# Lqm26/BMCNet-ESR

Measured on AMD Instinct MI355X. Metric: LR-voxel-frames/sec x4 SR train step, NFS-shaped 180x240 (BASELINE configs[1] / [2]), f32, higher is better.
Workload: dtype f32; 1 GPU; BMCNet(scale=4, n_c=128, n_b=5) x4 SR train step, NFS-shaped 180x240 (BASELINE configs[1] / [2]) -> 720x960, bs=4/GPU, arithmetic fp32 (native fp32 MFMA; 3x3 convolutions through Winograd F(4x4,3x3) / F(2x2,3x3) transforms in fp32), SEQL=9 SEQN=2 (8 windows BPTT), event scatter + fwd + MSE + bwd + Adam(amsgrad); global_batch=4, parallelism=dp1, rccl_ranks=1, rccl_initialised_before_headline_run=False

## Files before the change

### bmcnet-esr_amd/bmc_hip/bie.py

```python
from __future__ import annotations

import ctypes as C
import os
import weakref

import torch

from . import lib, ops
from .ops import ConvSpec, _dense_spec, _need_gpu, _null_src, _src, _stream, conv_launch, dgrad_launch, pgemm_raw, round_up

_SPEC2 = {}

FUSE_CHAIN = os.environ.get("BMC_FUSE_CHAIN", "1") != "0"
_CHAIN_CACHE = {}



VFREE = os.environ.get("BMC_BIE_VFREE", "1") != "0"
VFREE_MIN_PIXELS = int(os.environ.get("BMC_BIE_VFREE_MIN_PIXELS", 1 << 16))


def vfree_supported(npx):
    return VFREE and ops.MATH in (0, 3) and npx >= VFREE_MIN_PIXELS


def _gram_on_x(c_src, x_src, B, H, W, Cn, dev):
    slabs, nsplit, G, bsl = pgemm_raw(c_src, [x_src], B, H, W, 1, 1, Cn, Cn, dev, flops=2.0 * B * H * W * Cn * Cn, want_bias=True)
    G0 = torch.empty((B, Cn, Cn), device=dev, dtype=torch.float32)
    sc = torch.empty((B, Cn), device=dev, dtype=torch.float32)
    lib.call(lib._red_w, "bmc_pgemm_reduce_weight", slabs.data_ptr(), nsplit, G, 1, Cn, Cn, None, Cn, G0.data_ptr(), 0,
             bsl.data_ptr(), sc.data_ptr(), _stream())
    return G0, sc


def _times_wt(m, vec, wg, bg, bpg, alpha, out):
    B, Cn, _ = m.shape
    ops.small_mm([((m, Cn * Cn, 0, Cn, 1), (wg, 0, Cn * Cn, 1, Cn), None)], B, bpg, Cn, Cn, Cn, c=(out, Cn * Cn, 0, Cn, 1),
                 alpha=alpha, uv=((vec, Cn, 0), (bg, 0, Cn)))
    return out


def _times_w(m, wg, bg, bpg, out, out_strides, vec=None):
    B, Cn, _ = m.shape
    ops.small_mm([((m, Cn * Cn, 0, Cn, 1), (wg, 0, Cn * Cn, Cn, 1), (bg, 0, Cn, 1) if vec is not None else None)], B, bpg, Cn, Cn, Cn,
                 c=(out, out_strides[0], 0, out_strides[1], out_strides[2]), vec_out=(vec, Cn, 0) if vec is not None else None)


def _value_param_grads(p, dM, tg, da, G0, sc, w_params, b_params, npx):
    groups = len(w_params)
    B, Cn, _ = p.shape
    n, cc, dev = B // groups, Cn * Cn, p.device
    mp = round_up(Cn, 32)
    slab, bslab = groups * mp * mp, groups * 4 * mp
    slabs = torch.empty(n * slab, device=dev, dtype=torch.float32)
    bsl = torch.zeros(n * bslab, device=dev, dtype=torch.float32)
    params = list(w_params) + list(b_params)
    with ops.wgrad_side(npx, params, (p, dM, tg, da, G0, sc)):
        ops._on_side(slabs, bsl)
        ops.small_mm([((p, cc, 0, 1, Cn), (dM, cc, 0, Cn, 1), (tg, Cn, 0, 1)), ((da, cc, 0, 1, Cn), (G0, cc, 0, Cn, 1), (sc, Cn, 0, 1))],
                     B, n, Cn, Cn, Cn, c=(slabs, slab, mp * mp - n * slab, mp, 1), vec_out=(bsl, bslab, 4 * mp - n * bslab))
        one = groups == 1
        return ops.reduce_wgrad(slabs, n, groups, 1, Cn, _dense_spec(Cn), dev, bsl, w_params[0] if one else tuple(w_params),
                                b_params[0] if one else tuple(b_params), (Cn, Cn) if one else (groups, Cn, Cn))


def chain_supported(Cn):
    return FUSE_CHAIN and ops.MATH in (0, 3) and Cn in (32, 64, 128)


def _chain_streams(wf, wc, Cn):
    key = (id(wf), id(wc))
    hit = _CHAIN_CACHE.get(key)
    if hit is not None and hit[0]() is wf and hit[1]() is wc and hit[2] == (wf._version, wc._version):
        return hit[3], hit[4]
    dev = wf.device
    s1, s2 = _dense_spec(Cn), _spec2(Cn)
    st = _stream()

    def pack(w, spec, cin):
        out = torch.empty(spec.kpad * Cn, device=dev, dtype=torch.float32)
        lib.call(lib._pack_w, "bmc_pack_weight", w.data_ptr(), spec.kmap(dev).data_ptr(), 1, Cn, cin, 1, spec.kpad, Cn,
                 out.data_ptr(), st)
        return out

    def pack_t(w, spec, cin, src_index):
        out = torch.empty(Cn * Cn, device=dev, dtype=torch.float32)
        lib.call(lib._pack_wt, "bmc_pack_weight_t", w.data_ptr(), spec.kmap(dev).data_ptr(), 1, Cn, cin, 1,
                 src_index * Cn, Cn, Cn, Cn, out.data_ptr(), st)
        return out

    wfd, wcd = wf.detach().contiguous(), wc.detach().contiguous()
    fwd = torch.cat([pack(wfd, s2, 2 * Cn), pack(wcd, s1, Cn)])
    tc, t0, t1 = pack_t(wcd, s1, Cn, 0), pack_t(wfd, s2, 2 * Cn, 0), pack_t(wfd, s2, 2 * Cn, 1)
    bwd = torch.cat([tc, tc, t1, t1, t0])
    if len(_CHAIN_CACHE) > 64:
        for k in [k for k, v in _CHAIN_CACHE.items() if v[0]() is None or v[1]() is None]:
            del _CHAIN_CACHE[k]
    _CHAIN_CACHE[key] = (weakref.ref(wf), weakref.ref(wc), (wf._version, wc._version), fwd, bwd)
    return fwd, bwd


def chain_fwd(s0, s1, wf, bf, gamma, beta, wc, bc, eps, B, H, W, Cn, dev):
    fwd, _ = _chain_streams(wf, wc, Cn)
    yhat = torch.empty((B, H, W, Cn), device=dev, dtype=torch.float32)
    centre = torch.empty((B, H, W, Cn), device=dev, dtype=torch.float32)
    rstd = torch.empty(B * H * W, device=dev, dtype=torch.float32)
    a = lib.ChainFwdArgs()
    a.s0, a.s1 = s0, s1
    a.wstream = fwd.data_ptr()
    a.bias_f, a.bias_c, a.gamma, a.beta = bf.data_ptr(), bc.data_ptr(), gamma.data_ptr(), beta.data_ptr()
    a.eps = eps
    a.yhat, a.rstd, a.centre = yhat.data_ptr(), rstd.data_ptr(), centre.data_ptr()
    a.B, a.C, a.H, a.W = B, Cn, H, W
    e0 = ops._prof_begin()
    lib.call(lib._chain_fwd, "bmc_chain_fwd", C.byref(a), _stream())
    ops._prof_end(e0, "chain_kernel<fwd>", 2.0 * B * H * W * Cn * 3 * Cn, B * H * W * (16.0 * Cn + 4))
    return yhat, rstd, centre


def chain_bwd(dc, yhat, rstd, gamma, wf, wc, add, n, H, W, Cn, dev, ds1=None):
    _, bwd = _chain_streams(wf, wc, Cn)
    dz = torch.empty((2 * n, H, W, Cn), device=dev, dtype=torch.float32)
    if ds1 is None:
        ds1 = torch.empty((2 * n, H, W, Cn), device=dev, dtype=torch.float32)
    ds0 = torch.empty((n, H, W, Cn), device=dev, dtype=torch.float32)
    a = lib.ChainBwdArgs()
    a.dcentre = dc
    a.wstream = bwd.data_ptr()
    a.gamma, a.yhat, a.rstd = gamma.data_ptr(), yhat.data_ptr(), rstd.data_ptr()
    a.dz, a.ds1, a.ds0 = dz.data_ptr(), ds1.data_ptr(), ds0.data_ptr()
    a.ds0_add = add if add is not None else _null_src()
    a.n, a.C, a.H, a.W = n, Cn, H, W
    e0 = ops._prof_begin()
    lib.call(lib._chain_bwd, "bmc_chain_bwd", C.byref(a), _stream())
    ops._prof_end(e0, "chain_kernel<bwd>", 2.0 * 2 * n * H * W * Cn * 3 * Cn, 2 * n * H * W * (20.0 * Cn + 4))
    return dz, ds1, ds0


def _spec2(c):
    s = _SPEC2.get(c)
    if s is None:
        s = ConvSpec.dense(c, c)
        _SPEC2[c] = s
    return s


class BIETwinFn(torch.autograd.Function):

    @staticmethod
    def forward(ctx, x12, xs, rw1, rb1, rw2, rb2, wf, bf, gamma, beta, wc, bc, wu, bu, wv1, bv1, wv2, bv2, scale, eps):
        _need_gpu(x12)
        x12, xs = x12.contiguous(), xs.contiguous()
        B2, H, W, Cn = x12.shape
        n = B2 // 2
        dev = x12.device
        s1, s2 = _dense_spec(Cn), _spec2(Cn)
        new = lambda b: torch.empty((b, H, W, Cn), device=dev, dtype=torch.float32)
        X = lambda t, **k: _src(t, 0, Cn, k.get("shift", 0), k.get("mod"), k.get("b0", 0), k.get("B", t.shape[0]))
        d = lambda t: t.detach()
        t12, r12 = new(B2), new(B2)
        conv_launch([X(x12)], d(rw1).reshape(1, Cn, Cn, 9), s1, rw1, d(rb1), t12, B2, relu=True, rule=rb1)
        conv_launch([X(t12)], d(rw2).reshape(1, Cn, Cn, 9), s1, rw2, d(rb2), r12, B2, residual=X(x12), rule=rb2)
        fused = chain_supported(Cn)
        if fused:
            z12, stats, c12 = chain_fwd(X(xs, mod=n, B=B2), X(x12, shift=n, mod=B2), wf, d(bf), d(gamma), d(beta), wc, d(bc),
                                        eps, B2, H, W, Cn, dev)
            y12 = z12
        else:
            z12, y12, c12 = new(B2), new(B2), new(B2)
            conv_launch([X(xs, mod=n, B=B2), X(x12, shift=n, mod=B2)], d(wf).reshape(1, Cn, 2 * Cn, 1), s2, wf, d(bf), z12, B2)
            stats = torch.empty(B2 * H * W * 2, device=dev, dtype=torch.float32)
            lib.call(lib._ln_fwd, "bmc_layernorm_fwd", z12.data_ptr(), gamma.data_ptr(), beta.data_ptr(), B2 * H * W, Cn, eps,
                     y12.data_ptr(), stats.data_ptr(), _stream())
            conv_launch([X(y12)], d(wc).reshape(1, Cn, Cn, 1), s1, wc, d(bc), c12, B2)
        wv = ops.stacked((wv1, wv2), lambda: torch.stack([d(wv1).reshape(Cn, Cn, 1), d(wv2).reshape(Cn, Cn, 1)]), "v1x1")
        bv = ops.stacked((bv1, bv2), lambda: torch.stack([d(bv1), d(bv2)]), "stack")
        vfree = vfree_supported(B2 * H * W)
        o12 = new(B2)
        if vfree:
            G0, sc = _gram_on_x(X(c12), X(x12), B2, H, W, Cn, dev)
            wg, v12 = wv.view(2, Cn, Cn), None
            att = _times_wt(G0, sc, wg, bv, n, scale, torch.empty_like(G0))
            p = torch.empty_like(att)
            lib.call(lib._sm_fwd, "bmc_softmax_fwd", att.data_ptr(), B2 * Cn, Cn, p.data_ptr(), _stream())
            pw, pb = torch.empty_like(p), torch.empty_like(sc)
            _times_w(p, wg, bv, n, pw, (Cn * Cn, Cn, 1), vec=pb)
            conv_launch([X(x12)], pw.view(B2, Cn, Cn, 1), s1, None, pb, o12, B2, residual=X(r12, shift=n, mod=B2), bpg=1)
        else:
            G0 = sc = None
            v12 = new(B2)
            conv_launch([X(x12)], wv, s1, wv, bv, v12, B2, bpg=n)
            slabs, nsplit, G = pgemm_raw(X(c12), [X(v12)], B2, H, W, 1, 1, Cn, Cn, dev, flops=2.0 * B2 * H * W * Cn * Cn)
            att = torch.empty((B2, Cn, Cn), device=dev, dtype=torch.float32)
            lib.call(lib._red_p, "bmc_pgemm_reduce_plain", slabs.data_ptr(), nsplit, G, Cn, Cn, scale, att.data_ptr(), _stream())
            p = torch.empty_like(att)
            lib.call(lib._sm_fwd, "bmc_softmax_fwd", att.data_ptr(), B2 * Cn, Cn, p.data_ptr(), _stream())
            conv_launch([X(v12)], p.view(B2, Cn, Cn, 1), s1, None, None, o12, B2, residual=X(r12, shift=n, mod=B2), bpg=1)
        xs_new = new(n)
        conv_launch([X(c12, b0=0, B=n), X(c12, b0=n, B=n)], d(wu).reshape(1, Cn, 2 * Cn, 1), s2, wu, d(bu), xs_new, n, residual=X(xs))
        ctx.save_for_backward(x12, xs, t12, z12, stats, y12, c12, v12 if not vfree else G0, p, rw1, rw2, wf, gamma, wc, wu, wv1, wv2, beta,
                              *((sc, bv1, bv2) if vfree else ()))
        ctx.vfree = vfree
        ctx.owners = (rw1, rw2, wf, wc, wu)
        ctx.window = ops.current_window()
        ctx.params = (rw1, rb1, rw2, rb2, wf, bf, gamma, beta, wc, bc, wu, bu)
        ctx.vparams = (wv1, wv2, bv1, bv2)
        ctx.scale = scale
        ctx.fused = fused
        ctx.gslot = getattr(x12, "_bmc_gslot", None)
        return o12, xs_new

    @staticmethod
    def backward(ctx, do12, dxs_new):
        saved = ctx.saved_tensors
        x12, xs, t12, z12, stats, y12, c12, v12, p, rw1, rw2, wf, gamma, wc, wu, wv1, wv2, beta = saved[:18]
        vfree = ctx.vfree
        if vfree:
            G0, (sc, bv1, bv2) = v12, saved[18:]
        o_rw1, o_rw2, o_wf, o_wc, o_wu = ctx.owners
        p_rw1, p_rb1, p_rw2, p_rb2, p_wf, p_bf, p_gamma, p_beta, p_wc, p_bc, p_wu, p_bu = ctx.params
        B2, H, W, Cn = x12.shape
        n = B2 // 2
        dev = x12.device
        s1, s2 = _dense_spec(Cn), _spec2(Cn)
        new = lambda b: torch.empty((b, H, W, Cn), device=dev, dtype=torch.float32)
        X = lambda t, **k: _src(t, 0, Cn, k.get("shift", 0), k.get("mod"), k.get("b0", 0), k.get("B", t.shape[0]))
        g_o = do12.contiguous() if do12 is not None else torch.zeros_like(x12)
        g_x = dxs_new.contiguous() if dxs_new is not None else torch.zeros_like(xs)
        w_r1, w_r2 = rw1.detach().reshape(1, Cn, Cn, 9), rw2.detach().reshape(1, Cn, Cn, 9)
        w_f, w_c, w_u = (rw.detach().reshape(1, Cn, k, 1) for rw, k in ((wf, 2 * Cn), (wc, Cn), (wu, 2 * Cn)))
        w_v = ops.stacked(ctx.vparams[:2], lambda: torch.stack([wv1.detach().reshape(Cn, Cn, 1), wv2.detach().reshape(Cn, Cn, 1)]), "v1x1")

        if vfree:
            wg = w_v.view(2, Cn, Cn)
            bg = ops.stacked(ctx.vparams[2:], lambda: torch.stack([bv1.detach(), bv2.detach()]), "stack")
            dM, tg = _gram_on_x(X(g_o), X(x12), B2, H, W, Cn, dev)
            dp = _times_wt(dM, tg, wg, bg, n, 1.0, torch.empty_like(dM))
        else:
            slabs, nsplit, G = pgemm_raw(X(g_o), [X(v12)], B2, H, W, 1, 1, Cn, Cn, dev, flops=2.0 * B2 * H * W * Cn * Cn)
            dp = torch.empty_like(p)
            lib.call(lib._red_p, "bmc_pgemm_reduce_plain", slabs.data_ptr(), nsplit, G, Cn, Cn, 1.0, dp.data_ptr(), _stream())
        da = torch.empty_like(p)
        lib.call(lib._sm_bwd, "bmc_softmax_bwd", p.data_ptr(), dp.data_ptr(), B2 * Cn, Cn, ctx.scale, da.data_ptr(), _stream())
        if vfree:
            dwv, dbv = _value_param_grads(p, dM, tg, da, G0, sc, ctx.vparams[:2], ctx.vparams[2:], B2 * H * W)
        dc12 = new(B2)
        w_ut = ops.stacked((p_wu,), lambda: wu.detach().view(Cn, 2, Cn).permute(1, 2, 0).repeat_interleave(n, 0).contiguous(), "wut%d" % n)
        if vfree:
            w_dx = torch.empty((B2, Cn, 2 * Cn, 1), device=dev, dtype=torch.float32)
            w_dc = torch.empty((B2, Cn, 2 * Cn, 1), device=dev, dtype=torch.float32)
            w_dc.view(B2, Cn, 2 * Cn)[:, :, Cn:] = w_ut
            ds = torch.empty((B2, Cn), device=dev, dtype=torch.float32)
            cc2 = 2 * Cn * Cn
            _times_w(da, wg, bg, n, w_dc, (cc2, 2 * Cn, 1), vec=ds)
            _times_w(da, wg, bg, n, w_dx[:, :, Cn:], (cc2, 1, 2 * Cn))
            _times_w(p, wg, bg, n, w_dx, (cc2, 1, 2 * Cn))
            conv_launch([X(x12), X(g_x, mod=n, B=B2)], w_dc, s2, None, ds, dc12, B2, bpg=1)
        else:
            dv12 = new(B2)
            w_dv = torch.cat([p.transpose(1, 2), da.transpose(1, 2)], 2).view(B2, Cn, 2 * Cn, 1)
            conv_launch([X(g_o), X(c12)], w_dv, s2, None, None, dv12, B2, bpg=1)
            w_dc = torch.cat([da, w_ut], 2).view(B2, Cn, 2 * Cn, 1)
            conv_launch([X(v12), X(g_x, mod=n, B=B2)], w_dc, s2, None, None, dc12, B2, bpg=1)
        dwu, dbu = ops.wgrad(X(g_x), [X(c12, b0=0, B=n), X(c12, b0=n, B=n)], s2, n, H, W, 1, Cn, dev, p_wu, p_bu, keep=(g_x, c12), window=ctx.window, merge_pgemm=True)
        if not vfree:
            dwv, dbv = ops.wgrad(X(dv12), [X(x12)], s1, B2, H, W, 1, Cn, dev, ctx.vparams[:2], ctx.vparams[2:], G=2,
                              w_shape=(2, Cn, Cn, 1, 1), keep=(dv12, x12), window=ctx.window, merge_pgemm=True)
        if ctx.fused:
            dz12, dx12, dxs = chain_bwd(X(dc12), y12, stats, gamma.detach(), wf, wc, X(g_x), n, H, W, Cn, dev,
                                        ds1=ops.grad_slot(ctx.gslot, x12))
            Gm, dbc_t = ops.wgrad(X(dc12), [X(y12)], s1, B2, H, W, 1, Cn, dev, None, None, w_shape=(Cn, Cn), merge_pgemm=True)
            sg = ops.sink_group([p_wc, p_bc, p_gamma, p_beta])
            if sg is not None:
                (o_w, o_b, o_g, o_bt), acc = sg
                dwc = dbc = dgamma = dbeta = None
            else:
                o_w, o_b, acc = Gm, None, 0
                o_g = dgamma = torch.empty(Cn, device=dev, dtype=torch.float32)
                o_bt = dbeta = torch.empty(Cn, device=dev, dtype=torch.float32)
                dwc, dbc = Gm, dbc_t
            lib.call(lib._chain_affine, "bmc_chain_affine_grads", Gm.data_ptr(), dbc_t.data_ptr(), wc.detach().data_ptr(),
                     gamma.detach().data_ptr(), beta.detach().data_ptr(), Cn, o_w.data_ptr(),
                     o_b.data_ptr() if o_b is not None else None, o_g.data_ptr(), o_bt.data_ptr(), acc, _stream())
            dwf, dbf = ops.wgrad(X(dz12), [X(xs, mod=n, B=B2), X(x12, shift=n, mod=B2)], s2, B2, H, W, 1, Cn, dev, p_wf, p_bf,
                              keep=(dz12, xs, x12), window=ctx.window, merge_pgemm=True)
            if vfree:
                conv_launch([X(g_o), X(c12)], w_dx, s2, None, None, dx12, B2, bpg=1, accumulate=True)
            else:
                dgrad_launch(X(dv12), w_v, s1, 0, w_v, dx12, B2, bpg=n, accumulate=True)
        else:
            dx12 = ops.grad_slot(ctx.gslot, x12)
            if vfree:
                conv_launch([X(g_o), X(c12)], w_dx, s2, None, None, dx12, B2, bpg=1)
            else:
                dgrad_launch(X(dv12), w_v, s1, 0, w_v, dx12, B2, bpg=n)
            dwc, dbc = ops.wgrad(X(dc12), [X(y12)], s1, B2, H, W, 1, Cn, dev, p_wc, p_bc, keep=(dc12, y12), window=ctx.window, merge_pgemm=True)
            dy12 = new(B2)
            dgrad_launch(X(dc12), w_c, s1, 0, o_wc, dy12, B2)
            dz12 = new(B2)
            ws = torch.empty(2 * 1024 * Cn, device=dev, dtype=torch.float32)
            sg = ops.sink_group([p_gamma, p_beta])
            if sg is not None:
                (o_g, o_bt), ln_acc = sg
                dgamma = dbeta = None
            else:
                o_g = dgamma = torch.empty(Cn, device=dev, dtype=torch.float32)
                o_bt = dbeta = torch.empty(Cn, device=dev, dtype=torch.float32)
                ln_acc = 0
            lib.call(lib._ln_bwd, "bmc_layernorm_bwd", dy12.data_ptr(), z12.data_ptr(), stats.data_ptr(), gamma.data_ptr(),
                     B2 * H * W, Cn, dz12.data_ptr(), ws.data_ptr(), o_g.data_ptr(), o_bt.data_ptr(), ln_acc, _stream())
            dwf, dbf = ops.wgrad(X(dz12), [X(xs, mod=n, B=B2), X(x12, shift=n, mod=B2)], s2, B2, H, W, 1, Cn, dev, p_wf, p_bf,
                              keep=(dz12, xs, x12), window=ctx.window, merge_pgemm=True)
            dxs = new(n)
            dgrad_launch(X(dz12, b0=0, B=n), w_f, s2, 0, o_wf, dxs, n, residual=X(g_x))
            dgrad_launch(X(dz12, b0=n, B=n), w_f, s2, 0, o_wf, dxs, n, accumulate=True)
            dgrad_launch(X(dz12, shift=n, mod=B2), w_f, s2, 1, o_wf, dx12, B2, accumulate=True)
        g_r = X(g_o, shift=n, mod=B2)
        dw2, db2 = ops.wgrad(g_r, [X(t12)], s1, B2, H, W, 9, Cn, dev, p_rw2, p_rb2, keep=(g_o, t12), window=ctx.window, merge_pgemm=True)
        dt = new(B2)
        dgrad_launch(g_r, w_r2, s1, 0, o_rw2, dt, B2, mask=X(t12))
        dw1, db1 = ops.wgrad(X(dt), [X(x12)], s1, B2, H, W, 9, Cn, dev, p_rw1, p_rb1, keep=(dt, x12), window=ctx.window, merge_pgemm=True)
        dgrad_launch(X(dt), w_r1, s1, 0, o_rw1, dx12, B2, residual=g_r, accumulate=True)
        v = lambda t, ref: None if t is None else t.view(ref.shape)
        gv = (None,) * 4 if dwv is None else (dwv[0].reshape(wv1.shape), dbv[0], dwv[1].reshape(wv2.shape), dbv[1])
        return (dx12, dxs, dw1, db1, dw2, db2, dwf, dbf, dgamma, dbeta, v(dwc, wc), dbc, dwu, dbu, *gv, None, None)


class BIEFirstFn(torch.autograd.Function):

    @staticmethod
    def forward(ctx, x12, xs, rw1, rb1, rw2, rb2, wf, bf, gamma, beta, wc, bc, wu, bu, wv1, bv1, scale, eps):
        _need_gpu(x12)
        x12, xs = x12.contiguous(), xs.contiguous()
        B2, H, W, Cn = x12.shape
        n = B2 // 2
        dev = x12.device
        s1, s2 = _dense_spec(Cn), _spec2(Cn)
        new = lambda b: torch.empty((b, H, W, Cn), device=dev, dtype=torch.float32)
        X = lambda t, **k: _src(t, 0, Cn, k.get("shift", 0), k.get("mod"), k.get("b0", 0), k.get("B", t.shape[0]))
        d = lambda t: t.detach()
        second = X(x12, b0=n, B=n)
        t2, r2 = new(n), new(n)
        conv_launch([second], d(rw1).reshape(1, Cn, Cn, 9), s1, rw1, d(rb1), t2, n, relu=True, rule=rb1)
        conv_launch([X(t2)], d(rw2).reshape(1, Cn, Cn, 9), s1, rw2, d(rb2), r2, n, residual=second, rule=rb2)
        yhat, rstd, c12 = chain_fwd(X(xs, mod=n, B=B2), X(x12, shift=n, mod=B2), wf, d(bf), d(gamma), d(beta), wc, d(bc), eps,
                                    B2, H, W, Cn, dev)
        vfree = vfree_supported(B2 * H * W)
        o1 = new(n)
        if vfree:
            G0, sc = _gram_on_x(X(c12, b0=0, B=n), X(x12, b0=0, B=n), n, H, W, Cn, dev)
            wg, bg, v1 = d(wv1).reshape(1, Cn, Cn), d(bv1).reshape(1, Cn), None
            att = _times_wt(G0, sc, wg, bg, n, scale, torch.empty_like(G0))
            p = torch.empty_like(att)
            lib.call(lib._sm_fwd, "bmc_softmax_fwd", att.data_ptr(), n * Cn, Cn, p.data_ptr(), _stream())
            pw, pb = torch.empty_like(p), torch.empty_like(sc)
            _times_w(p, wg, bg, n, pw, (Cn * Cn, Cn, 1), vec=pb)
            conv_launch([X(x12, b0=0, B=n)], pw.view(n, Cn, Cn, 1), s1, None, pb, o1, n, residual=X(r2), bpg=1)
        else:
            G0 = sc = None
            v1 = new(n)
            conv_launch([X(x12, b0=0, B=n)], d(wv1).reshape(1, Cn, Cn, 1), s1, wv1, d(bv1), v1, n)
            slabs, nsplit, G = pgemm_raw(X(c12, b0=0, B=n), [X(v1)], n, H, W, 1, 1, Cn, Cn, dev, flops=2.0 * n * H * W * Cn * Cn)
            att = torch.empty((n, Cn, Cn), device=dev, dtype=torch.float32)
            lib.call(lib._red_p, "bmc_pgemm_reduce_plain", slabs.data_ptr(), nsplit, G, Cn, Cn, scale, att.data_ptr(), _stream())
            p = torch.empty_like(att)
            lib.call(lib._sm_fwd, "bmc_softmax_fwd", att.data_ptr(), n * Cn, Cn, p.data_ptr(), _stream())
            conv_launch([X(v1)], p.view(n, Cn, Cn, 1), s1, None, None, o1, n, residual=X(r2), bpg=1)
        xs_new = new(n)
        conv_launch([X(c12, b0=0, B=n), X(c12, b0=n, B=n)], d(wu).reshape(1, Cn, 2 * Cn, 1), s2, wu, d(bu), xs_new, n, residual=X(xs))
        ctx.save_for_backward(x12, xs, t2, yhat, rstd, c12, v1 if not vfree else G0, p, rw1, rw2, wf, gamma, wc, wu, wv1, beta,
                              *((sc, bv1) if vfree else ()))
        ctx.vfree = vfree
        ctx.owners = (rw1, rw2, wf, wc, wu, wv1)
        ctx.window = ops.current_window()
        ctx.params = (rw1, rb1, rw2, rb2, wf, bf, gamma, beta, wc, bc, wu, bu, wv1, bv1)
        ctx.scale = scale
        return o1, xs_new

    @staticmethod
    def backward(ctx, do1, dxs_new):
        saved = ctx.saved_tensors
        x12, xs, t2, yhat, rstd, c12, v1, p, rw1, rw2, wf, gamma, wc, wu, wv1, beta = saved[:16]
        vfree = ctx.vfree
        if vfree:
            G0, (sc, bv1) = v1, saved[16:]
        o_rw1, o_rw2, o_wf, o_wc, o_wu, o_wv1 = ctx.owners
        p_rw1, p_rb1, p_rw2, p_rb2, p_wf, p_bf, p_gamma, p_beta, p_wc, p_bc, p_wu, p_bu, p_wv1, p_bv1 = ctx.params
        B2, H, W, Cn = x12.shape
        n = B2 // 2
        dev = x12.device
        s1, s2 = _dense_spec(Cn), _spec2(Cn)
        new = lambda b: torch.empty((b, H, W, Cn), device=dev, dtype=torch.float32)
        X = lambda t, **k: _src(t, 0, Cn, k.get("shift", 0), k.get("mod"), k.get("b0", 0), k.get("B", t.shape[0]))
        g_o = do1.contiguous() if do1 is not None else torch.zeros_like(t2)
        g_x = dxs_new.contiguous() if dxs_new is not None else torch.zeros_like(xs)
        w_r1, w_r2 = rw1.detach().reshape(1, Cn, Cn, 9), rw2.detach().reshape(1, Cn, Cn, 9)
        w_v1 = wv1.detach().reshape(1, Cn, Cn, 1)
        if vfree:
            wg, bg = wv1.detach().reshape(1, Cn, Cn), bv1.detach().reshape(1, Cn)
            dM, tg = _gram_on_x(X(g_o), X(x12, b0=0, B=n), n, H, W, Cn, dev)
            dp = _times_wt(dM, tg, wg, bg, n, 1.0, torch.empty_like(dM))
        else:
            slabs, nsplit, G = pgemm_raw(X(g_o), [X(v1)], n, H, W, 1, 1, Cn, Cn, dev, flops=2.0 * n * H * W * Cn * Cn)
            dp = torch.empty_like(p)
            lib.call(lib._red_p, "bmc_pgemm_reduce_plain", slabs.data_ptr(), nsplit, G, Cn, Cn, 1.0, dp.data_ptr(), _stream())
        da = torch.empty_like(p)
        lib.call(lib._sm_bwd, "bmc_softmax_bwd", p.data_ptr(), dp.data_ptr(), n * Cn, Cn, ctx.scale, da.data_ptr(), _stream())
        if vfree:
            dwv1, dbv1 = _value_param_grads(p, dM, tg, da, G0, sc, (p_wv1,), (p_bv1,), n * H * W)
            if dwv1 is not None:
                dwv1, dbv1 = dwv1.view(wv1.shape), dbv1.view(Cn)
        dc12 = new(B2)
        w_ut = ops.stacked((p_wu,), lambda: wu.detach().view(Cn, 2, Cn).permute(1, 2, 0).repeat_interleave(n, 0).contiguous(), "wut%d" % n)
        if vfree:
            w_dx = torch.empty((n, Cn, 2 * Cn, 1), device=dev, dtype=torch.float32)
            w_dc = torch.zeros((B2, Cn, 2 * Cn, 1), device=dev, dtype=torch.float32)
            w_dc.view(B2, Cn, 2 * Cn)[:, :, Cn:] = w_ut
            ds = torch.zeros((B2, Cn), device=dev, dtype=torch.float32)
            cc2 = 2 * Cn * Cn
            _times_w(da, wg, bg, n, w_dc, (cc2, 2 * Cn, 1), vec=ds)
            _times_w(da, wg, bg, n, w_dx[:, :, Cn:], (cc2, 1, 2 * Cn))
            _times_w(p, wg, bg, n, w_dx, (cc2, 1, 2 * Cn))
            conv_launch([X(x12), X(g_x, mod=n, B=B2)], w_dc, s2, None, ds, dc12, B2, bpg=1)
        else:
            dv1 = new(n)
            w_dv = torch.cat([p.transpose(1, 2), da.transpose(1, 2)], 2).view(n, Cn, 2 * Cn, 1)
            conv_launch([X(g_o), X(c12, b0=0, B=n)], w_dv, s2, None, None, dv1, n, bpg=1)
            w_dc = torch.cat([torch.cat([da, torch.zeros_like(da)], 0), w_ut], 2).view(B2, Cn, 2 * Cn, 1)
            conv_launch([X(v1, mod=n, B=B2), X(g_x, mod=n, B=B2)], w_dc, s2, None, None, dc12, B2, bpg=1)
        dwu, dbu = ops.wgrad(X(g_x), [X(c12, b0=0, B=n), X(c12, b0=n, B=n)], s2, n, H, W, 1, Cn, dev, p_wu, p_bu, keep=(g_x, c12), window=ctx.window, merge_pgemm=True)
        if not vfree:
            dwv1, dbv1 = ops.wgrad(X(dv1), [X(x12, b0=0, B=n)], s1, n, H, W, 1, Cn, dev, p_wv1, p_bv1, keep=(dv1, x12), window=ctx.window, merge_pgemm=True)
        dz12, dx12, dxs = chain_bwd(X(dc12), yhat, rstd, gamma.detach(), wf, wc, X(g_x), n, H, W, Cn, dev)
        Gm, dbc_t = ops.wgrad(X(dc12), [X(yhat)], s1, B2, H, W, 1, Cn, dev, None, None, w_shape=(Cn, Cn), merge_pgemm=True)
        sg = ops.sink_group([p_wc, p_bc, p_gamma, p_beta])
        if sg is not None:
            (o_w, o_b, o_g, o_bt), acc = sg
            dwc = dbc = dgamma = dbeta = None
        else:
            o_w, o_b, acc = Gm, None, 0
            o_g = dgamma = torch.empty(Cn, device=dev, dtype=torch.float32)
            o_bt = dbeta = torch.empty(Cn, device=dev, dtype=torch.float32)
            dwc, dbc = Gm, dbc_t
        lib.call(lib._chain_affine, "bmc_chain_affine_grads", Gm.data_ptr(), dbc_t.data_ptr(), wc.detach().data_ptr(),
                 gamma.detach().data_ptr(), beta.detach().data_ptr(), Cn, o_w.data_ptr(),
                 o_b.data_ptr() if o_b is not None else None, o_g.data_ptr(), o_bt.data_ptr(), acc, _stream())
        dwf, dbf = ops.wgrad(X(dz12), [X(xs, mod=n, B=B2), X(x12, shift=n, mod=B2)], s2, B2, H, W, 1, Cn, dev, p_wf, p_bf,
                          keep=(dz12, xs, x12), window=ctx.window, merge_pgemm=True)
        if vfree:
            conv_launch([X(g_o), X(c12, b0=0, B=n)], w_dx, s2, None, None, dx12, n, bpg=1, accumulate=True)
        else:
            dgrad_launch(X(dv1), w_v1, s1, 0, o_wv1, dx12, n, accumulate=True)
        dw2, db2 = ops.wgrad(X(g_o), [X(t2)], s1, n, H, W, 9, Cn, dev, p_rw2, p_rb2, keep=(g_o, t2), window=ctx.window, merge_pgemm=True)
        dt = new(n)
        dgrad_launch(X(g_o), w_r2, s1, 0, o_rw2, dt, n, mask=X(t2))
        dw1, db1 = ops.wgrad(X(dt), [X(x12, b0=n, B=n)], s1, n, H, W, 9, Cn, dev, p_rw1, p_rb1, keep=(dt, x12), window=ctx.window, merge_pgemm=True)
        dgrad_launch(X(dt), w_r1, s1, 0, o_rw1, dx12, n, residual=X(g_o), accumulate=True, out_b0=n)
        v = lambda t, ref: None if t is None else t.view(ref.shape)
        return (dx12, dxs, dw1, db1, dw2, db2, dwf, dbf, dgamma, dbeta, v(dwc, wc), dbc, dwu, dbu, v(dwv1, wv1), dbv1, None, None)


def bie_first(m, x12, xs):
    r = m.conv1
    return BIEFirstFn.apply(x12, xs, r.conv1.weight, r.conv1.bias, r.conv2.weight, r.conv2.bias, m.convf1.weight,
                            m.convf1.bias, m.norm_s.weight, m.norm_s.bias, m.clustering.weight, m.clustering.bias,
                            m.unclustering.weight, m.unclustering.bias, m.v1.weight, m.v1.bias, m.scale, m.norm_s.eps)


def bie_twin(m, x12, xs):
    r = m.conv1
    return BIETwinFn.apply(x12, xs, r.conv1.weight, r.conv1.bias, r.conv2.weight, r.conv2.bias, m.convf1.weight,
                           m.convf1.bias, m.norm_s.weight, m.norm_s.bias, m.clustering.weight, m.clustering.bias,
                           m.unclustering.weight, m.unclustering.bias, m.v1.weight, m.v1.bias, m.v2.weight, m.v2.bias,
                           m.scale, m.norm_s.eps)


class Stack2Fn(torch.autograd.Function):

    @staticmethod
    def forward(ctx, a, b, slot):
        buf, n = slot.t, a.shape[0]
        assert a.data_ptr() == buf.data_ptr() and b.data_ptr() == buf[n:].data_ptr() and buf.shape[0] == 2 * n
        ctx.n = n
        return buf

    @staticmethod
    def backward(ctx, g):
        return g[:ctx.n], g[ctx.n:], None


class Unstack2Fn(torch.autograd.Function):

    @staticmethod
    def forward(ctx, t, n=None):
        n = t.shape[0] // 2 if n is None else n
        ctx.n = n
        ctx.shape = t.shape
        return t[:n], t[n:]

    @staticmethod
    def unstack(t):
        a, b = Unstack2Fn.apply(t)
        if t.requires_grad and a.grad_fn is not None:
            pair = ops.GradPair(t.shape[0] // 2, t.shape)
            a._bmc_gslot, b._bmc_gslot = (pair, 0), (pair, 1)
            a.grad_fn.pair = pair
        return a, b

    @staticmethod
    def backward(ctx, g1, g2):
        if g1 is not None and g2 is not None and g1.is_contiguous() and g2.is_contiguous() \
                and g1.untyped_storage().data_ptr() == g2.untyped_storage().data_ptr() \
                and g2.storage_offset() == g1.storage_offset() + g1.numel():
            out = torch.empty(0, device=g1.device, dtype=g1.dtype)
            out.set_(g1.untyped_storage(), g1.storage_offset(), tuple(ctx.shape), torch.empty(ctx.shape, device="meta").stride())
            pair = getattr(ctx, "pair", None)
            if pair is not None:
                pair.buf = None
            return out, None
        pair = getattr(ctx, "pair", None)
        if pair is not None:
            pair.buf = None
        z = lambda k: torch.zeros((k,) + tuple(ctx.shape[1:]), device=(g1 if g1 is not None else g2).device)
        return torch.cat([g1 if g1 is not None else z(ctx.n), g2 if g2 is not None else z(ctx.shape[0] - ctx.n)], 0), None
```

### bmcnet-esr_amd/bmc_hip/lib.py

```python
from __future__ import annotations

import ctypes as C
import os

import torch

_HERE = os.path.dirname(os.path.abspath(__file__))
LIB_PATH = os.environ.get("BMC_HIP_LIB") or os.path.join(os.path.dirname(_HERE), "csrc", "libbmc_hip.so")

if not os.path.exists(LIB_PATH):
    raise ImportError(
        f"{LIB_PATH} not found: build the HIP extension first "
        "(python -c 'import __graft_entry__ as g; g.build()' or make -C bmcnet-esr_amd/csrc). "
        "The BMCNet MI355X path has no CPU fallback.")

_lib = C.CDLL(LIB_PATH)

MAX_SRC = 6
c_fp = C.c_void_p


class Src(C.Structure):
    _fields_ = [("ptr", C.c_void_p), ("batch_stride", C.c_longlong), ("pix_stride", C.c_int), ("nch", C.c_int),
                ("batch_shift", C.c_int), ("batch_mod", C.c_int)]


class ConvArgs(C.Structure):
    _fields_ = [("nsrc", C.c_int), ("src", Src * MAX_SRC), ("wpacked", C.c_void_p), ("bias", C.c_void_p),
                ("w_group_stride", C.c_longlong), ("bias_group_stride", C.c_int), ("batch_per_group", C.c_int),
                ("out", C.c_void_p), ("out_batch_stride", C.c_longlong), ("out_pix_stride", C.c_int),
                ("B", C.c_int), ("H", C.c_int), ("W", C.c_int), ("Cout", C.c_int), ("Coutpad", C.c_int),
                ("taps", C.c_int), ("relu", C.c_int), ("residual", Src), ("mask", Src), ("accumulate", C.c_int),
                ("math", C.c_int)]


class PgemmArgs(C.Structure):
    _fields_ = [("a", Src), ("nsrc", C.c_int), ("src", Src * MAX_SRC), ("B", C.c_int), ("H", C.c_int), ("W", C.c_int),
                ("taps", C.c_int), ("batch_per_group", C.c_int), ("slabs", C.c_void_p), ("nsplit", C.c_int),
                ("zeros", C.c_void_p), ("bias_slabs", C.c_void_p), ("math", C.c_int), ("tap_groups", C.c_int)]


class ChainFwdArgs(C.Structure):
    _fields_ = [("s0", Src), ("s1", Src), ("wstream", C.c_void_p), ("bias_f", C.c_void_p), ("bias_c", C.c_void_p),
                ("gamma", C.c_void_p), ("beta", C.c_void_p), ("eps", C.c_float), ("yhat", C.c_void_p), ("rstd", C.c_void_p),
                ("centre", C.c_void_p), ("B", C.c_int), ("C", C.c_int), ("H", C.c_int), ("W", C.c_int)]


class ChainBwdArgs(C.Structure):
    _fields_ = [("dcentre", Src), ("wstream", C.c_void_p), ("gamma", C.c_void_p), ("yhat", C.c_void_p), ("rstd", C.c_void_p),
                ("dz", C.c_void_p), ("ds1", C.c_void_p), ("ds0", C.c_void_p), ("ds0_add", Src), ("n", C.c_int), ("C", C.c_int),
                ("H", C.c_int), ("W", C.c_int)]


class MmTerm(C.Structure):
    _fields_ = [("a", C.c_void_p), ("a_sb", C.c_longlong), ("a_sg", C.c_longlong), ("a_si", C.c_int), ("a_sk", C.c_int),
                ("b", C.c_void_p), ("b_sb", C.c_longlong), ("b_sg", C.c_longlong), ("b_sk", C.c_int), ("b_sj", C.c_int),
                ("w", C.c_void_p), ("w_sb", C.c_longlong), ("w_sg", C.c_longlong), ("w_sk", C.c_int)]


class SmallMmArgs(C.Structure):
    _fields_ = [("nterms", C.c_int), ("t", MmTerm * 2), ("nbatch", C.c_int), ("batch_per_group", C.c_int),
                ("M", C.c_int), ("N", C.c_int), ("K", C.c_int), ("alpha", C.c_float),
                ("u", C.c_void_p), ("u_sb", C.c_longlong), ("u_sg", C.c_longlong),
                ("v", C.c_void_p), ("v_sb", C.c_longlong), ("v_sg", C.c_longlong),
                ("c", C.c_void_p), ("c_sb", C.c_longlong), ("c_sg", C.c_longlong), ("c_si", C.c_int), ("c_sj", C.c_int),
                ("vec_out", C.c_void_p), ("vo_sb", C.c_longlong), ("vo_sg", C.c_longlong), ("accumulate", C.c_int)]


def _sig(name, argtypes, restype=C.c_int):
    fn = getattr(_lib, name)
    fn.argtypes = argtypes
    fn.restype = restype
    return fn


_ll, _i, _f, _p = C.c_longlong, C.c_int, C.c_float, C.c_void_p

bmc_version = _sig("bmc_version", [])
bmc_last_error = _sig("bmc_last_error", [], C.c_char_p)
_events = _sig("bmc_events_to_channels", [_p, _p, _p, _p, _i, _i, _i, _p, _i, _p])
_voxel = _sig("bmc_events_to_voxel", [_p, _p, _p, _p, _p, _ll, _i, _i, _i, _i, _p, _i, _p, _p])
_stack_pol = _sig("bmc_events_to_stack_polarity", [_p, _p, _p, _p, _ll, _p, _p, _i, _i, _i, _p, _p, _i, _p])
_mask = _sig("bmc_events_to_mask", [_p, _p, _p, _ll, _i, _i, _p, _p, _i, _p])
_stack = _sig("bmc_events_to_stack", [_p, _p, _p, _p, _ll, _p, _p, _i, _i, _i, _p, _p, _i, _p])
_enc_raw = _sig("bmc_encode_raw_events", [_p, _p, _p, _p, _p, _i, _i, _i, _p, _p])
_events_ws = _sig("bmc_events_binned_ws_bytes", [_ll, _i, _i, _i], C.c_longlong)
_events_binned = _sig("bmc_events_to_channels_binned", [_p, _p, _p, _p, _ll, _i, _i, _i, _p, _i, _p, _ll, _p])
_enc_raw_binned = _sig("bmc_encode_raw_events_binned", [_p, _p, _p, _p, _p, _ll, _i, _i, _i, _p, _p, _ll, _p])
_ev_torch_ws = _sig("bmc_events_torch_ws_ints", [_ll, _i, _i], C.c_longlong)
_ev_img_torch = _sig("bmc_events_to_image_torch", [_p, _p, _p, _ll, _i, _i, _i, _i, _i, _p, _p, _p])
_ev_vox_torch = _sig("bmc_events_to_voxel_torch", [_p, _p, _p, _p, _ll, _i, _i, _i, _p, _p, _p])
_pack_w = _sig("bmc_pack_weight", [_p, _p, _i, _i, _i, _i, _i, _i, _p, _p])
_pack_wt = _sig("bmc_pack_weight_t", [_p, _p, _i, _i, _i, _i, _i, _i, _i, _i, _p, _p])
_pack_wino = _sig("bmc_pack_weight_wino", [_p, _p, _i, _i, _i, _i, _i, _i, _i, _i, _p, _p])
_pack_wino4 = _sig("bmc_pack_weight_wino4", [_p, _p, _i, _i, _i, _i, _i, _i, _i, _i, _p, _p])
_ww_nsplit = _sig("bmc_wgrad_wino_nsplit", [_i, _i, _i])
_stream_low = _sig("bmc_stream_create_low_priority", [C.POINTER(C.c_void_p)])
_small_mm = _sig("bmc_small_mm", [C.POINTER(SmallMmArgs), _p])
_ww = _sig("bmc_wgrad_wino", [C.POINTER(Src), C.POINTER(Src), _i, _i, _i, _i, _p, _p, _p])
_ww_red = _sig("bmc_wgrad_wino_reduce", [_p, _i, _p, _i, _i, _i, _p, _p, _p])
_ww_multi = _sig("bmc_wgrad_wino_multi", [C.POINTER(Src), C.POINTER(Src), C.POINTER(C.c_int), _i, _i, _i, _i, _p, _p, _p])
_ptr_table = _sig("bmc_ptr_table", [C.POINTER(C.c_ulonglong), _i, _p, _p])
_wino_rows = _sig("bmc_conv_wino_rows", [_i, _i, _i, _i, _i])
_ww4_nsplit = _sig("bmc_wgrad_wino4_nsplit", [_i, _i, _i])
_ww4 = _sig("bmc_wgrad_wino4", [C.POINTER(Src), C.POINTER(Src), _i, _i, _i, _i, _p, _p, _p])
_ww4_red = _sig("bmc_wgrad_wino4_reduce", [_p, _i, _p, _i, _i, _i, _p, _p, _p])
_split_w = _sig("bmc_split_weight", [_p, _p, _ll, _i, _i, _p])
_conv = _sig("bmc_conv", [C.POINTER(ConvArgs), _p])
_pgemm = _sig("bmc_pgemm", [C.POINTER(PgemmArgs), _p])
pgemm_wave_map = _sig("bmc_pgemm_wave_map", [_i, _i, _i])
_red_w = _sig("bmc_pgemm_reduce_weight", [_p, _i, _i, _i, _i, _i, _p, _i, _p, _i, _p, _p, _p])
_red_wg = _sig("bmc_pgemm_reduce_weight_groups", [_p, _i, _i, _i, _i, _i, _p, _i, _p, _i, _p, _p, _p])
_red_p = _sig("bmc_pgemm_reduce_plain", [_p, _i, _i, _i, _i, _f, _p, _p])
_colsum = _sig("bmc_colsum", [_p, _ll, _i, _i, _p, _p, _i, _p])
_relu_bwd = _sig("bmc_relu_bwd", [_p, _p, _p, _ll, _p])
_ln_fwd = _sig("bmc_layernorm_fwd", [_p, _p, _p, _ll, _i, _f, _p, _p, _p])
_ln_bwd = _sig("bmc_layernorm_bwd", [_p, _p, _p, _p, _ll, _i, _p, _p, _p, _p, _i, _p])
_sm_fwd = _sig("bmc_softmax_fwd", [_p, _ll, _i, _p, _p])
_sm_bwd = _sig("bmc_softmax_bwd", [_p, _p, _ll, _i, _f, _p, _p])
_pack_in = _sig("bmc_pack_inputs", [_p, _ll, _ll, _ll, _ll, _ll, _i, _i, _i, _i, _p, _p, _p])
_unshuffle = _sig("bmc_unshuffle_to_nhwc", [_p, _i, _i, _i, _i, _i, _p, _i, _p])
_shuffle = _sig("bmc_shuffle_to_hr", [_p, _i, _i, _i, _i, _i, _p, _ll, _ll, _ll, _ll, _p, _i, _p])
_head_mse_fwd = _sig("bmc_head_mse_fwd", [_p, _i, _i, _i, _i, _i, _p, _ll, _ll, _ll, _ll, _p, _ll, _p, _p, _p, _p])
_head_mse_bwd = _sig("bmc_head_mse_bwd", [_p, _p, _p, _ll, _p, _i, _i, _i, _i, _i, _p, _p])
_group_sum = _sig("bmc_group_sum", [_p, _i, _ll, _p, _p])
_bicubic_fwd = _sig("bmc_bicubic_resize_fwd", [_p, _ll, _i, _i, _i, _i, _p, _p])
_bicubic_bwd = _sig("bmc_bicubic_resize_bwd", [_p, _ll, _i, _i, _i, _i, _p, _p])
_chain_fwd = _sig("bmc_chain_fwd", [C.POINTER(ChainFwdArgs), _p])
_chain_bwd = _sig("bmc_chain_bwd", [C.POINTER(ChainBwdArgs), _p])
_chain_affine = _sig("bmc_chain_affine_grads", [_p, _p, _p, _p, _p, _i, _p, _p, _p, _p, _i, _p])
_slot_stage = _sig("bmc_slot_stage", [_p, _i, _i, _i, _i, _p, _p, _i, _p, _i, _ll, _p, _ll, _p])
_slot_commit = _sig("bmc_slot_commit", [_p, _i, C.POINTER(C.c_void_p), _i, _ll, _p, _i, _p, _p, _ll, _p])
_slot_metrics = _sig("bmc_slot_metrics", [_p, _i, _p, _i, _i, _i, _i, _i, _i, _i, _p])
_slot_encode = _sig("bmc_slot_encode", [_p, _i, _i, _i, _i, _i, _i, _p, _p, _p])
_slot_emit = _sig("bmc_slot_emit", [_p, _p, _i, _p, _i, _i, _i, _i, _p, _p])
_slot_emit_timed = _sig("bmc_slot_emit_timed", [_p, _p, _i, _p, _i, _i, _i, _i, _p, _p, _p, _ll, _p])
_slot_emit_clocked = _sig("bmc_slot_emit_clocked", [_p, _p, _p, _i, _p, _i, _i, _i, _i, _p, _p, _p, _ll, _p])
_slot_emit_timed_ws = _sig("bmc_slot_emit_timed_scratch_bytes", [_i, _i, _ll], C.c_longlong)
_slot_hot_update = _sig("bmc_slot_hot_update", [_p, _p, _i, _i, _i, _i, _i, _i, _p, _p, _p, _p])
_slot_encode_filtered = _sig("bmc_slot_encode_filtered", [_p, _p, _p, _i, _i, _i, _i, _i, _i, _p, _p, _p])
_hot_pixel_mask = _sig("bmc_hot_pixel_mask", [_p, _i, _i, _i, _i, _f, _p, _p, _p])
_slot_render = _sig("bmc_slot_render", [_p, _p, _i, _i, _i, _i, _i, _p, _p])

EXPORTS = ["bmc_version", "bmc_last_error", "bmc_events_to_channels", "bmc_events_to_voxel", "bmc_events_to_stack", "bmc_encode_raw_events", "bmc_pack_weight", "bmc_pack_weight_t", "bmc_split_weight", "bmc_conv",
           "bmc_pgemm", "bmc_pgemm_wave_map", "bmc_pgemm_reduce_weight", "bmc_pgemm_reduce_plain", "bmc_colsum", "bmc_relu_bwd",
           "bmc_layernorm_fwd", "bmc_layernorm_bwd", "bmc_softmax_fwd", "bmc_softmax_bwd", "bmc_pack_inputs",
           "bmc_unshuffle_to_nhwc", "bmc_shuffle_to_hr", "bmc_bicubic_resize_fwd", "bmc_bicubic_resize_bwd",
           "bmc_chain_fwd", "bmc_chain_bwd", "bmc_chain_affine_grads", "bmc_group_sum",
           "bmc_head_mse_fwd", "bmc_head_mse_bwd", "bmc_events_to_stack_polarity", "bmc_events_to_mask",
           "bmc_pgemm_reduce_weight_groups", "bmc_events_binned_ws_bytes", "bmc_events_to_channels_binned",
           "bmc_encode_raw_events_binned", "bmc_pack_weight_wino", "bmc_pack_weight_wino4", "bmc_wgrad_wino_nsplit", "bmc_wgrad_wino",
           "bmc_wgrad_wino_reduce", "bmc_events_torch_ws_ints", "bmc_events_to_image_torch",
           "bmc_events_to_voxel_torch", "bmc_stream_create_low_priority", "bmc_small_mm",
           "bmc_wgrad_wino4_nsplit", "bmc_wgrad_wino4", "bmc_wgrad_wino4_reduce", "bmc_wgrad_wino_multi", "bmc_ptr_table",
           "bmc_conv_wino_rows", "bmc_slot_stage", "bmc_slot_commit", "bmc_slot_metrics", "bmc_slot_encode", "bmc_slot_emit",
           "bmc_slot_emit_timed", "bmc_slot_emit_timed_scratch_bytes", "bmc_slot_emit_clocked", "bmc_slot_hot_update",
           "bmc_slot_encode_filtered", "bmc_hot_pixel_mask", "bmc_slot_render"]


def check(rc, what):
    if rc != 0:
        raise RuntimeError(f"{what} failed (rc={rc}): {bmc_last_error().decode()}")


def call(fn, what, *args):
    check(fn(*args), what)


def has_symbol(name: str) -> bool:
    return hasattr(_lib, name)
```

### bmcnet-esr_amd/bmc_hip/ops.py

```python
from __future__ import annotations

import ctypes as C
import os
import threading
import weakref
from collections import namedtuple
from typing import List, Optional, Sequence

import torch

from . import lib

CK = 16
_cur_dev = torch._C._cuda_getDevice


_STREAM_OVERRIDE = None
_STREAM_OVERRIDE_TS = None


def _stream():
    if _STREAM_OVERRIDE is not None:
        return _STREAM_OVERRIDE
    return torch._C._cuda_getCurrentRawStream(_cur_dev())


def _on_side(*tensors):
    if _STREAM_OVERRIDE is not None:
        for t in tensors:
            if t is not None:
                t.record_stream(_STREAM_OVERRIDE_TS)


def _need_gpu(t: torch.Tensor):
    if not t.is_cuda:
        raise RuntimeError("bmc_hip: tensor is on %s -- the BMCNet MI355X path has no CPU fallback" % t.device)
    if t.dtype != torch.float32:
        raise RuntimeError("bmc_hip: fp32 tensors only (got %s)" % t.dtype)
    if t.device.index != _cur_dev():
        raise RuntimeError("bmc_hip: tensor lives on %s but the current device is cuda:%d -- call torch.cuda.set_device "
                           "(one process per GPU)" % (t.device, _cur_dev()))


def round_up(v, m):
    return (v + m - 1) // m * m


def coutpad(c):
    return 32 if c <= 32 else round_up(c, 128)


class View:
    __slots__ = ("t", "c0", "nch", "shift", "mod", "b0")

    def __init__(self, t, c0=0, nch=None, shift=0, mod=None, b0=0):
        self.t = t
        self.c0 = c0
        self.nch = t.shape[3] - c0 if nch is None else nch
        self.shift = shift
        self.mod = mod
        self.b0 = b0

    def meta(self):
        return (self.c0, self.nch, self.shift, self.mod, self.b0)


def _src(t: torch.Tensor, c0, nch, shift, mod, b0, launch_b) -> lib.Src:
    Bt, H, W, Ct = t.shape
    s = lib.Src()
    s.ptr = t.data_ptr() + 4 * (b0 * H * W * Ct + c0)
    s.batch_stride = H * W * Ct
    s.pix_stride = Ct
    s.nch = nch
    s.batch_shift = shift
    s.batch_mod = mod if mod is not None else max(launch_b, 1) + shift
    return s


def _null_src() -> lib.Src:
    s = lib.Src()
    s.ptr = None
    s.batch_mod = 1
    return s


class ConvSpec:

    def __init__(self, sources: Sequence[Sequence[int]], cin: Optional[int] = None):
        self.nch = [len(s) for s in sources]
        for n in self.nch:
            assert n % CK == 0, "source channel windows must be multiples of 16"
        flat = [c for s in sources for c in s]
        self.kpad = len(flat)
        self.kmap_host = flat
        self.cin = max(flat) + 1 if cin is None else cin
        assert self.cin > max(flat)
        self.covers_all = set(range(self.cin)) <= set(flat)
        self.kreal = sum(1 for c in flat if c >= 0)
        self.real_nch = [sum(1 for c in src if c >= 0) for src in sources]
        self._kmap = {}
        self._packs = {}

    def kmap(self, device):
        k = self._kmap.get(device)
        if k is None:
            k = torch.tensor(self.kmap_host, dtype=torch.int32, device=device)
            self._kmap[device] = k
        return k

    @staticmethod
    def dense(*nchs):
        out, c = [], 0
        for n in nchs:
            out.append(list(range(c, c + n)))
            c += n
        return ConvSpec(out)



PROFILE = None
PROFILE_WINO = [0, 0]


def _prof_record(e):
    if _STREAM_OVERRIDE is not None:
        e.record(_STREAM_OVERRIDE_TS)
    else:
        e.record()


def _prof_begin():
    if PROFILE is None:
        return None
    e = torch.cuda.Event(enable_timing=True)
    _prof_record(e)
    return e


def _prof_end(e0, kind, flops, nbytes=0.0):
    if e0 is not None:
        e1 = torch.cuda.Event(enable_timing=True)
        _prof_record(e1)
        PROFILE.append((kind, flops, e0, e1, nbytes))


MATH_NAMES = {"fp32": 0, "bf16": 1, "bf16x6": 3}
MATH = MATH_NAMES[os.environ.get("BMC_MATH", "fp32")]


def set_math(mode):
    global MATH
    MATH = MATH_NAMES[mode] if isinstance(mode, str) else int(mode)
    if MATH not in (0, 1, 3):
        raise ValueError("unknown math mode %r" % (mode,))


def _split_planes(packed: torch.Tensor, cp: int):
    nsteps = packed.numel() // (cp * CK)
    out = torch.empty(nsteps * MATH * cp * (CK // 2), device=packed.device, dtype=torch.int32)
    lib.call(lib._split_w, "bmc_split_weight", packed.data_ptr(), out.data_ptr(), nsteps, cp, MATH, _stream())
    return out


def _cache_get(spec: ConvSpec, kind, owner):
    if owner is None:
        return None
    hit = spec._packs.get((kind, id(owner)))
    if hit is not None and hit[0]() is owner and hit[1] == (owner._version, _EPOCH):
        return hit[2]
    return None


def _cache_put(spec: ConvSpec, kind, owner, packed):
    if owner is not None:
        if len(spec._packs) > 64:
            for k in [k for k, v in spec._packs.items() if v[0]() is None]:
                del spec._packs[k]
        spec._packs[(kind, id(owner))] = (weakref.ref(owner), (owner._version, _EPOCH), packed)


_STACKS = {}


def invalidate_caches():
    global _EPOCH
    _EPOCH += 1
    _STACKS.clear()
    from . import bie
    bie._CHAIN_CACHE.clear()


_EPOCH = 0


def stacked(owners, build, tag=""):
    key = (tag,) + tuple(id(o) for o in owners)
    vers = tuple(o._version for o in owners)
    hit = _STACKS.get(key)
    if hit is not None and hit[1] == vers and all(r() is o for r, o in zip(hit[0], owners)):
        return hit[2]
    t = build()
    if len(_STACKS) > 256:
        for k in [k for k, v in _STACKS.items() if any(r() is None for r in v[0])]:
            del _STACKS[k]
    _STACKS[key] = (tuple(weakref.ref(o) for o in owners), vers, t)
    return t


WINO = os.environ.get("BMC_WINO", "1") != "0"
WINO_MIN_TILES = int(os.environ.get("BMC_WINO_MIN_TILES", 128))


WINO4 = os.environ.get("BMC_WINO4", "1") != "0"
WINO4_MIN_TILES = int(os.environ.get("BMC_WINO4_MIN_TILES", 300))

_EXACT_ZERO = threading.local()
DENSE_FLOOR = 1e-5
_DENSE = {}


class exact_zero_inputs:
    def __enter__(self):
        _EXACT_ZERO.n = getattr(_EXACT_ZERO, "n", 0) + 1

    def __exit__(self, *exc):
        _EXACT_ZERO.n -= 1
        return False


class dense_inputs:
    def __enter__(self):
        _EXACT_ZERO.d = getattr(_EXACT_ZERO, "d", 0) + 1

    def __exit__(self, *exc):
        _EXACT_ZERO.d -= 1
        return False


def _dense_cached(b):
    hit = _DENSE.get(id(b))
    if hit is not None and hit[0]() is b and hit[1] == b._version:
        return hit
    return None


def prime_bias_dense(biases):
    need = [b for b in biases if b is not None and _dense_cached(b) is None]
    if not need or not need[0].is_cuda or torch.cuda.is_current_stream_capturing():
        return
    vals = torch.stack([torch.stack((b.detach().abs().min(), b.detach().max())) for b in need]).tolist()
    if len(_DENSE) > 512:
        for k in [k for k, v in _DENSE.items() if v[0]() is None]:
            del _DENSE[k]
    for b, (mn, mx) in zip(need, vals):
        _DENSE[id(b)] = (weakref.ref(b), b._version, mn, mx)


def _bias_entry(b):
    hit = _dense_cached(b)
    if hit is None:
        prime_bias_dense([b])
        hit = _dense_cached(b)
    return hit


def bias_dense(b):
    if b is None:
        return False
    if isinstance(b, (tuple, list)):
        prime_bias_dense(b)
        return all(bias_dense(x) for x in b)
    hit = _bias_entry(b)
    return hit is not None and hit[2] >= DENSE_FLOOR


def bias_positive(b):
    if b is None:
        return False
    if isinstance(b, (tuple, list)):
        prime_bias_dense(b)
        return all(bias_positive(x) for x in b)
    hit = _bias_entry(b)
    return hit is not None and hit[3] >= DENSE_FLOOR


_WINO_ROWS = {}
WINO_MIN_TILES4 = int(os.environ.get("BMC_WINO_MIN_TILES4", 128))


def wino_tiles(B, H, W, cp):
    key = (B, H, W, cp)
    th = _WINO_ROWS.get(key)
    if th is None:
        th = _WINO_ROWS[key] = lib._wino_rows(B, H, W, cp, 0)
    return B * ((H + th - 1) // th) * ((W + 15) // 16) * (cp // 128), th


def wino_ok(B, H, W, Cout, taps, fwd=False, stride=0, rule=None):
    if not WINO or MATH != 0 or taps != 9:
        return 0
    cp = coutpad(Cout)
    if cp % 128:
        return 0
    nt, th = wino_tiles(B, H, W, cp)
    if nt < (WINO_MIN_TILES if th == 8 else min(WINO_MIN_TILES, WINO_MIN_TILES4)):
        return 0
    if H * W * 4 * max(stride, 512) >= 2 ** 31:
        return 0
    if WINO4 and W >= 17 and H * W < 2 ** 24:
        n4 = B * ((((H + 3) // 4) * ((W + 3) // 4) + 15) // 16) * (cp // 128)
        if n4 >= WINO4_MIN_TILES and not (fwd and (getattr(_EXACT_ZERO, "n", 0) or
                                                   not (getattr(_EXACT_ZERO, "d", 0) or bias_dense(rule)))):
            return 4
    return 2


PAIR_SMALL = os.environ.get("BMC_PAIR_SMALL", "1") != "0"
PAIR_ALWAYS = os.environ.get("BMC_PAIR_SMALL") == "2"
PAIR_BELOW_TILES = 200


def pair_small(B2, H, W):
    t = B2 * ((H + 7) // 8) * ((W + 15) // 16)
    return PAIR_SMALL and WINO and MATH == 0 and (PAIR_ALWAYS or t < PAIR_BELOW_TILES <= 2 * t)


def _packed_weight(w4: torch.Tensor, spec: ConvSpec, owner, wino=False):
    G, Cout, Cin, taps = w4.shape
    if wino:
        npos = 36 if wino == 4 else 16
        hit = _cache_get(spec, ("fw", npos), owner)
        if hit is not None:
            return hit
        cp = coutpad(Cout)
        out = torch.empty(G * spec.kpad * npos * cp, device=w4.device, dtype=torch.float32)
        fn, nm = (lib._pack_wino4, "bmc_pack_weight_wino4") if wino == 4 else (lib._pack_wino, "bmc_pack_weight_wino")
        lib.call(fn, nm, w4.data_ptr(), spec.kmap(w4.device).data_ptr(), G, Cout, Cin,
                 spec.kpad, cp, 0, 0, 0, out.data_ptr(), _stream())
        _cache_put(spec, ("fw", npos), owner, out)
        return out
    hit = _cache_get(spec, ("f", MATH), owner)
    if hit is not None:
        return hit
    cp = coutpad(Cout)
    out = torch.empty(G * spec.kpad * taps * cp, device=w4.device, dtype=torch.float32)
    lib.call(lib._pack_w, "bmc_pack_weight", w4.data_ptr(), spec.kmap(w4.device).data_ptr(), G, Cout, Cin, taps,
             spec.kpad, cp, out.data_ptr(), _stream())
    if MATH:
        out = _split_planes(out, cp)
    _cache_put(spec, ("f", MATH), owner, out)
    return out


def _packed_weight_t(w4: torch.Tensor, spec: ConvSpec, src_index: int, owner, wino=False):
    G, Cout, Cin, taps = w4.shape
    k0 = sum(spec.nch[:src_index])
    nk = spec.nch[src_index]
    nkpad = coutpad(nk)
    c16 = round_up(Cout, CK)
    if wino:
        npos = 36 if wino == 4 else 16
        hit = _cache_get(spec, ("tw", src_index, npos), owner)
        if hit is not None:
            return hit
        out = torch.empty(G * c16 * npos * nkpad, device=w4.device, dtype=torch.float32)
        fn, nm = (lib._pack_wino4, "bmc_pack_weight_wino4") if wino == 4 else (lib._pack_wino, "bmc_pack_weight_wino")
        lib.call(fn, nm, w4.data_ptr(), spec.kmap(w4.device).data_ptr(), G, Cout, Cin,
                 c16, nkpad, 1, k0, nk, out.data_ptr(), _stream())
        _cache_put(spec, ("tw", src_index, npos), owner, out)
        return out
    hit = _cache_get(spec, ("t", src_index, MATH), owner)
    if hit is not None:
        return hit
    out = torch.empty(G * c16 * taps * nkpad, device=w4.device, dtype=torch.float32)
    lib.call(lib._pack_wt, "bmc_pack_weight_t", w4.data_ptr(), spec.kmap(w4.device).data_ptr(), G, Cout, Cin, taps,
             k0, nk, nkpad, c16, out.data_ptr(), _stream())
    if MATH:
        out = _split_planes(out, nkpad)
    _cache_put(spec, ("t", src_index, MATH), owner, out)
    return out



def conv_raw(srcs: List[lib.Src], wpacked, w_group_stride, bias, bias_group_stride, out_ptr, out_batch_stride,
             out_pix_stride, B, H, W, Cout, taps, relu=False, residual: Optional[lib.Src] = None, bpg=None,
             accumulate=False, flops=0.0, mask: Optional[lib.Src] = None, wino=False):
    a = lib.ConvArgs()
    a.nsrc = len(srcs)
    for i, s in enumerate(srcs):
        a.src[i] = s
    a.wpacked = wpacked.data_ptr()
    a.bias = bias.data_ptr() if bias is not None else None
    a.w_group_stride = w_group_stride * MATH // 2 if MATH else w_group_stride
    a.math = MATH
    if wino:
        assert MATH == 0 and taps == 9
        a.w_group_stride = w_group_stride // 9 * (36 if wino == 4 else 16)
        a.math = 5 if wino == 4 else 4
    a.bias_group_stride = bias_group_stride
    a.batch_per_group = bpg if bpg else B
    a.out = out_ptr
    a.out_batch_stride = out_batch_stride
    a.out_pix_stride = out_pix_stride
    a.B, a.H, a.W = B, H, W
    a.Cout, a.Coutpad = Cout, coutpad(Cout)
    a.taps = taps
    a.relu = int(relu)
    a.residual = residual if residual is not None else _null_src()
    a.mask = mask if mask is not None else _null_src()
    a.accumulate = int(accumulate)
    e0 = _prof_begin()
    lib.call(lib._conv, "bmc_conv", C.byref(a), _stream())
    _prof_end(e0, ("wino4_conv<9,128>" if wino == 4 else "wino_conv<9,128>") if wino else
              "conv_kernel<%d,%d>" % (taps, 32 if a.Coutpad == 32 else 128), flops,
              4.0 * B * H * W * (sum(x.nch for x in srcs) + Cout * (1 + (residual is not None) + (mask is not None) + bool(accumulate))))
    if PROFILE is not None and e0 is not None:
        PROFILE_WINO[0 if wino else 1] += 1


_ZEROS = {}


def _zeros(device):
    z = _ZEROS.get(device)
    if z is None:
        z = torch.zeros(64, device=device, dtype=torch.float32)
        _ZEROS[device] = z
    return z


TAP_SPLIT_TILES = 8


def pgemm_raw(a_src: lib.Src, srcs: List[lib.Src], B, H, W, taps, bpg, M, N, device, flops=0.0, want_bias=False):
    G = B // bpg
    mpad, npad = round_up(M, 32), round_up(N, 32)
    if taps == 9:
        cols = 32 if MATH == 3 else 64
        n_nblk = (npad + cols - 1) // cols
        tiles = ((H + 3) // 4) * ((W + 15) // 16)
        target = 256
    else:
        n_nblk = (npad + 127) // 128
        tiles = (H * W + 63) // 64
        target = 256
    other = G * ((mpad + 127) // 128) * n_nblk
    nsplit = max(1, min(bpg * tiles, target // max(other, 1)))
    tap_groups = 1
    if taps == 9 and MATH in (0, 1) and bpg * tiles < TAP_SPLIT_TILES * nsplit and nsplit >= 3:
        tap_groups = 3
        nsplit = max(1, min(bpg * tiles, target // max(other * 3, 1)))
    slabs = torch.empty(nsplit * G * taps * mpad * npad, device=device, dtype=torch.float32)
    p = lib.PgemmArgs()
    p.a = a_src
    p.nsrc = len(srcs)
    for i, s in enumerate(srcs):
        p.src[i] = s
    p.B, p.H, p.W, p.taps = B, H, W, taps
    p.batch_per_group = bpg
    p.slabs = slabs.data_ptr()
    p.nsplit = nsplit
    p.zeros = _zeros(device).data_ptr()
    p.math = MATH
    p.tap_groups = tap_groups
    bslabs = None
    if want_bias:
        bslabs = torch.empty(nsplit * G * 4 * mpad, device=device, dtype=torch.float32)
        p.bias_slabs = bslabs.data_ptr()
    else:
        p.bias_slabs = None
    _on_side(slabs, bslabs)
    e0 = _prof_begin()
    lib.call(lib._pgemm, "bmc_pgemm", C.byref(p), _stream())
    _prof_end(e0, "pgemm_kernel<%d>" % taps, flops, 4.0 * B * H * W * (a_src.nch + sum(x.nch for x in srcs)) + 4.0 * slabs.numel())
    if want_bias:
        return slabs, nsplit, G, bslabs
    return slabs, nsplit, G


WINO_WGRAD = os.environ.get("BMC_WINO_WGRAD", "1") != "0"
WINO4_WGRAD = os.environ.get("BMC_WINO4_WGRAD", "1") != "0"
WINO4_WGRAD_MIN_STAGES = int(os.environ.get("BMC_WINO4_WGRAD_MIN_STAGES", 24))


def wgrad_wino4_ok(B, H, W):
    if not WINO4_WGRAD:
        return False
    stages = B * ((H + 3) // 4) * (((W + 3) // 4 + 3) // 4)
    return stages >= 32 * WINO4_WGRAD_MIN_STAGES


def wino_wgrad_ok(a_src, x_srcs, spec, taps, Cout, G):
    if not (WINO and WINO_WGRAD and MATH == 0 and taps == 9 and G == 1 and Cout == 128 and len(x_srcs) == 1 and spec.kpad == 128):
        return False
    xs = x_srcs[0]
    if not (xs.nch == 128 and xs.pix_stride == 128 and a_src.nch == 128 and a_src.pix_stride == 128):
        return False
    k0 = spec.kmap_host[0]
    return k0 >= 0 and spec.kmap_host == list(range(k0, k0 + 128))


WGRAD_MERGE = max(1, min(8, int(os.environ.get("BMC_WGRAD_MERGE", 5))))
WGRAD_MERGE_MAX_PIXELS = int(os.environ.get("BMC_WGRAD_MERGE_MAX_PIXELS", 1 << 17))


_WINDOW = [0]


def next_window():
    _WINDOW[0] += 1
    return _WINDOW[0]


def current_window():
    return _WINDOW[0]


_Use = namedtuple("_Use", "a_src x_srcs B keep")


class _MergeQueue:
    __slots__ = ("uses", "wino", "spec", "dev", "w_param", "b_param", "k0", "full", "H", "W", "taps", "Cout", "w_shape", "window")

    def __init__(self, **fields):
        self.uses = []
        for k, v in fields.items():
            setattr(self, k, v)


_MERGE = {}
_FLUSH_QUEUED = set()
PTR_TABLE_MAX = 256


def flush_wgrads(task=None):
    if task is None:
        task = torch._C._current_graph_task_id()
    _FLUSH_QUEUED.discard(task)
    qs = _MERGE.pop(task, None)
    if not qs:
        return
    for q in list(qs.values()):
        if q.uses:
            _launch_merged(q)


def _queue_flush(task):
    if task not in _FLUSH_QUEUED:
        _FLUSH_QUEUED.add(task)
        torch.autograd.Variable._execution_engine.queue_callback(lambda: flush_wgrads(task))


_TABLES = {}


def _table_src(srcs, batches, btot, dev):
    ptrs = []
    for s_, nb in zip(srcs, batches):
        mod = s_.batch_mod if s_.batch_mod >= 1 else 1
        ptrs.extend(s_.ptr + 4 * (((i + s_.batch_shift) % mod) * s_.batch_stride) for i in range(nb))
    st = _stream()
    key = (dev.index, st.value if hasattr(st, "value") else st, tuple(ptrs))
    table = _TABLES.get(key)
    if table is None:
        if len(_TABLES) >= 8192:
            _TABLES.clear()
        table = torch.empty(btot, device=dev, dtype=torch.int64)
        lib.call(lib._ptr_table, "bmc_ptr_table", (C.c_ulonglong * btot)(*ptrs), btot, table.data_ptr(), st)
        if not torch.cuda.is_current_stream_capturing():
            _TABLES[key] = table
    t = lib.Src()
    t.ptr = table.data_ptr()
    t.batch_stride, t.pix_stride, t.nch, t.batch_shift, t.batch_mod = 0, srcs[0].pix_stride, srcs[0].nch, 0, -1
    return t, table


def _launch_merged(q):
    uses, q.uses = q.uses, []
    keep = tuple(t for u in uses for t in u.keep)
    batches = [u.B for u in uses]
    npx = batches[0] * q.H * q.W
    want_bias = q.b_param is not None
    with wgrad_side(npx, [q.w_param, q.b_param], keep):
        if q.wino:
            _wgrad_wino([u.a_src for u in uses], [u.x_srcs[0] for u in uses], batches, q.H, q.W, q.spec, q.dev, q.w_param, q.b_param,
                        None, want_bias, q.k0, q.full)
            return
        btot = sum(batches)
        a_t, tab_a = _table_src([u.a_src for u in uses], batches, btot, q.dev)
        x_tt = [_table_src([u.x_srcs[k] for u in uses], batches, btot, q.dev) for k in range(len(uses[0].x_srcs))]
        _on_side(tab_a, *[tb for _, tb in x_tt])
        _pgemm_wgrad(a_t, [t for t, _ in x_tt], btot, q.H, q.W, q.taps, q.Cout, q.spec, q.dev, q.w_param, q.b_param, q.w_shape, 1, want_bias)


def _queue_use(wino, a_src, x_srcs, B, H, W, taps, Cout, spec, dev, w_param, b_param, w_shape, want_bias, k0, full, keep, window):
    task = torch._C._current_graph_task_id()
    if not (WGRAD_MERGE > 1 and window is not None and B * H * W <= WGRAD_MERGE_MAX_PIXELS and task >= 0 and w_param is not None
            and not isinstance(w_param, (tuple, list)) and is_sink(w_param) and (not want_bias or is_sink(b_param)) and keep
            and not torch.cuda.is_current_stream_capturing()):
        return False
    if wino:
        if wgrad_wino4_ok(B, H, W):
            return False
    elif not (B <= PTR_TABLE_MAX and a_src.batch_mod != -1 and all(x.batch_mod != -1 for x in x_srcs)):
        return False
    key = (id(w_param), k0, taps, len(x_srcs), H, W, want_bias)
    qs = _MERGE.setdefault(task, {})
    q = qs.get(key)
    if q is None or q.w_param is not w_param or q.window != window:
        if q is not None and q.uses:
            _launch_merged(q)
        q = qs[key] = _MergeQueue(wino=wino, spec=spec, dev=dev, w_param=w_param, b_param=b_param if want_bias else None, k0=k0,
                                  full=full, H=H, W=W, taps=taps, Cout=Cout, w_shape=w_shape, window=window)
    if not wino and q.uses and sum(u.B for u in q.uses) + B > PTR_TABLE_MAX:
        _launch_merged(q)
    _queue_flush(task)
    _side_arm(B * H * W)
    q.uses.append(_Use(a_src, list(x_srcs), B, tuple(keep)))
    if len(q.uses) >= WGRAD_MERGE:
        _launch_merged(q)
    return True


def _pgemm_wgrad(a_src, x_srcs, B, H, W, taps, Cout, spec, dev, w_param, b_param, w_shape, G, want_bias):
    r = pgemm_raw(a_src, x_srcs, B, H, W, taps, B // G, Cout, spec.kpad, dev, flops=2.0 * B * H * W * Cout * taps * spec.kreal,
                  want_bias=want_bias)
    return reduce_wgrad(r[0], r[1], G, taps, Cout, spec, dev, r[3] if want_bias else None, w_param, b_param if want_bias else None,
                        w_shape)


def wgrad_pgemm(a_src, x_srcs, B, H, W, taps, Cout, spec, dev, w_param, b_param, w_shape, G=1, want_bias=True, keep=(), window=None):
    want_bias = bool(want_bias)
    if G == 1 and _queue_use(False, a_src, x_srcs, B, H, W, taps, Cout, spec, dev, w_param, b_param, w_shape, want_bias, None,
                             spec.covers_all, keep, window):
        return None, None
    with wgrad_side(B * H * W, _flat_params(w_param, b_param if want_bias else None), keep):
        return _pgemm_wgrad(a_src, x_srcs, B, H, W, taps, Cout, spec, dev, w_param, b_param, w_shape, G, want_bias)


def wgrad_wino(a_src, x_src, B, H, W, spec, dev, w_param, b_param, w_shape, want_bias=True, k0=None, full=None, keep=(), window=None):
    want_bias = bool(want_bias)
    k0 = spec.kmap_host[0] if k0 is None else k0
    full = spec.covers_all if full is None else full
    if _queue_use(True, a_src, [x_src], B, H, W, 9, 128, spec, dev, w_param, b_param, w_shape, want_bias, k0, full, keep, window):
        return None, None
    with (wgrad_side(B * H * W, [w_param, b_param] if want_bias else [w_param], keep) if w_param is not None else _NOCTX):
        return _wgrad_wino([a_src], [x_src], [B], H, W, spec, dev, w_param, b_param, w_shape, want_bias, k0, full)


def _wgrad_wino(a_srcs, x_srcs, Bs, H, W, spec, dev, w_param, b_param, w_shape, want_bias, k0, full):
    n, Bt = len(a_srcs), sum(Bs)
    if n == 1 and wgrad_wino4_ok(Bt, H, W):
        f_ns, f_main, f_red, nm, npos, kind = lib._ww4_nsplit, lib._ww4, lib._ww4_red, "bmc_wgrad_wino4", 36, "wgrad_wino4<9>"
    else:
        f_ns, f_main, f_red, nm, npos, kind = lib._ww_nsplit, lib._ww, lib._ww_red, "bmc_wgrad_wino", 16, "wgrad_wino<9>"
    nsplit = f_ns(Bt, H, W)
    part = torch.empty(nsplit * npos * 128 * 128, device=dev, dtype=torch.float32)
    bpart = torch.empty(nsplit * 128, device=dev, dtype=torch.float32) if want_bias else None
    bpart_p = bpart.data_ptr() if want_bias else None
    _on_side(part, bpart)
    e0 = _prof_begin()
    if n > 1:
        lib.call(lib._ww_multi, "bmc_wgrad_wino_multi", (lib.Src * n)(*a_srcs), (lib.Src * n)(*x_srcs), (C.c_int * n)(*Bs), n, H, W, nsplit,
                 part.data_ptr(), bpart_p, _stream())
    else:
        lib.call(f_main, nm, C.byref(a_srcs[0]), C.byref(x_srcs[0]), Bt, H, W, nsplit, part.data_ptr(), bpart_p, _stream())
    _prof_end(e0, kind, 2.0 * Bt * H * W * 128 * 9 * 128, 4.0 * Bt * H * W * 256 + 4.0 * part.numel())
    sg = sink_group([w_param, b_param] if want_bias else [w_param], full) if w_param is not None else None
    if sg is not None:
        (gw, *rest), acc = sg
        lib.call(f_red, nm + "_reduce", part.data_ptr(), nsplit, gw.data_ptr(), spec.cin, k0, acc, bpart_p,
                 rest[0].data_ptr() if want_bias else None, _stream())
        return None, None
    assert n == 1
    dw = (torch.empty if full else torch.zeros)(128 * spec.cin * 9, device=dev, dtype=torch.float32)
    db = torch.empty(128, device=dev, dtype=torch.float32) if want_bias else None
    lib.call(f_red, nm + "_reduce", part.data_ptr(), nsplit, dw.data_ptr(), spec.cin, k0, 0, bpart_p,
             db.data_ptr() if want_bias else None, _stream())
    return dw.view(w_shape), db


def split_wgrad(spec, metas):
    cache = spec.__dict__.setdefault("_split", {})
    key = tuple(tuple(m) for m in metas)
    if key in cache:
        return cache[key] or None
    big, rest, off = [], [], 0
    for i, n in enumerate(spec.nch):
        seg = spec.kmap_host[off:off + n]
        c0, nch, shift, mod, b0 = metas[i]
        if n == 128 and nch == 128 and shift == 0 and mod is None and seg[0] >= 0 and seg == list(range(seg[0], seg[0] + 128)):
            big.append((i, seg[0]))
        else:
            rest.append(i)
        off += n
    res = False
    if big and len(spec.nch) > 1:
        sub = None
        if rest:
            offs = [sum(spec.nch[:i]) for i in range(len(spec.nch))]
            sub = ConvSpec([spec.kmap_host[offs[i]:offs[i] + spec.nch[i]] for i in rest], cin=spec.cin)
        res = (big, rest, sub)
    cache[key] = res
    return res or None


def wgrad_route(spec, a_src, x_srcs, metas, taps, Cout, G, w_param, b_param=None, want_bias=False):
    if not (WINO and WINO_WGRAD and MATH == 0 and taps == 9 and Cout == 128) or w_param is None:
        return "pgemm", None
    if isinstance(w_param, (tuple, list)):
        if (1 < G <= 4 and len(w_param) == G and metas is not None and metas[0][2] == 0 and metas[0][3] is None
                and wino_wgrad_ok(a_src, x_srcs, spec, taps, Cout, 1)):
            return "wino_groups", None
        return "pgemm", None
    if (G == 1 and len(x_srcs) > 1 and metas is not None and is_sink(w_param) and (not want_bias or is_sink(b_param))
            and a_src.pix_stride == 128 and all(x.pix_stride == 128 for x, n in zip(x_srcs, spec.nch) if n == 128)):
        sp = split_wgrad(spec, metas)
        if sp is not None:
            return "split", sp
    return ("wino" if wino_wgrad_ok(a_src, x_srcs, spec, taps, Cout, G) else "pgemm"), None


def _batch_window(s: lib.Src, b0, nb) -> lib.Src:
    w = lib.Src()
    w.ptr, w.batch_stride, w.pix_stride, w.nch = s.ptr + 4 * b0 * s.batch_stride, s.batch_stride, s.pix_stride, s.nch
    w.batch_shift, w.batch_mod = 0, max(nb, 1)
    return w


def wgrad(a_src, x_srcs, spec, B, H, W, taps, Cout, dev, w_param, b_param, G=1, w_shape=None, keep=(), window=None, *, metas=None,
          want_bias=True, merge_pgemm):
    if not want_bias:
        b_param = None
    if w_shape is None:
        w_shape = w_param.shape
    route, sp = wgrad_route(spec, a_src, x_srcs, metas, taps, Cout, G, w_param, b_param, want_bias)
    if route == "wino":
        return wgrad_wino(a_src, x_srcs[0], B, H, W, spec, dev, w_param, b_param, w_shape, want_bias=want_bias, keep=keep, window=window)
    if route == "split":
        big, rest, sub = sp
        for n, (i, k0) in enumerate(big):
            first = want_bias and n == 0
            wgrad_wino(a_src, x_srcs[i], B, H, W, spec, dev, w_param, b_param if first else None, w_shape, want_bias=first, k0=k0,
                       full=False, keep=(keep[0], keep[1 + i]), window=window)
        if rest:
            wgrad_pgemm(a_src, [x_srcs[i] for i in rest], B, H, W, taps, Cout, sub, dev, w_param, None, w_shape, want_bias=False, keep=keep)
        return None, None
    if route == "wino_groups":
        bpg = B // G
        outs = [wgrad_wino(_batch_window(a_src, gi * bpg, bpg), _batch_window(x_srcs[0], gi * bpg, bpg), bpg, H, W, spec, dev,
                           w_param[gi], b_param[gi] if want_bias else None, w_param[gi].shape, want_bias=want_bias, keep=keep,
                           window=window) for gi in range(G)]
        return [o[0] for o in outs], [o[1] for o in outs]
    return wgrad_pgemm(a_src, x_srcs, B, H, W, taps, Cout, spec, dev, w_param, b_param, w_shape, G=G, want_bias=want_bias, keep=keep,
                       window=window if merge_pgemm else None)


def _launch_stride(srcs, Co, residual, mask):
    return max([x.pix_stride for x in srcs] + [Co] + [x.pix_stride for x in (residual, mask) if x is not None])


def conv_launch(srcs, w4, spec, owner, bias, out, B, relu=False, residual=None, mask=None, bpg=None, accumulate=False,
                out_b0=0, rule=None):
    G, Cout, Cin, taps = w4.shape
    _, H, W, Co = out.shape
    wn = wino_ok(B, H, W, Cout, taps, fwd=not accumulate and mask is None, stride=_launch_stride(srcs, Co, residual, mask), rule=rule)
    wp = _packed_weight(w4, spec, owner, wino=wn)
    conv_raw(srcs, wp, spec.kpad * taps * coutpad(Cout), bias, Cout if bias is not None else 0,
             out.data_ptr() + 4 * out_b0 * H * W * Co, H * W * Co, Co, B, H, W, Cout, taps, relu=relu, residual=residual,
             bpg=bpg, accumulate=accumulate, mask=mask, flops=2.0 * B * H * W * Cout * taps * spec.kreal, wino=wn)


def dgrad_launch(g_src, w4, spec, src_index, owner, out, B, residual=None, mask=None, bpg=None, accumulate=False, out_b0=0, out_c0=0):
    G, Cout, Cin, taps = w4.shape
    _, H, W, Co = out.shape
    nch = spec.nch[src_index]
    wn = wino_ok(B, H, W, nch, taps, stride=_launch_stride([g_src], Co, residual, mask))
    wt = _packed_weight_t(w4, spec, src_index, owner, wino=wn)
    conv_raw([g_src], wt, round_up(Cout, CK) * taps * coutpad(nch), None, 0, out.data_ptr() + 4 * (out_b0 * H * W * Co + out_c0),
             H * W * Co, Co, B, H, W, nch, taps, residual=residual, mask=mask, bpg=bpg, accumulate=accumulate,
             flops=2.0 * B * H * W * spec.real_nch[src_index] * taps * Cout, wino=wn)


def relu_bwd(dy, y):
    g = torch.empty_like(dy)
    lib.call(lib._relu_bwd, "bmc_relu_bwd", dy.data_ptr(), y.data_ptr(), g.data_ptr(), dy.numel(), _stream())
    return g


def group_sum(g, groups):
    n = g.shape[0] // groups
    out = torch.empty((n,) + tuple(g.shape[1:]), device=g.device, dtype=torch.float32)
    lib.call(lib._group_sum, "bmc_group_sum", g.data_ptr(), groups, out.numel(), out.data_ptr(), _stream())
    return out


def colsum(x2d_ptr, npix, pix_stride, Cn, device):
    ws = torch.empty(2048 * Cn, device=device, dtype=torch.float32)
    out = torch.empty(Cn, device=device, dtype=torch.float32)
    lib.call(lib._colsum, "bmc_colsum", x2d_ptr, npix, pix_stride, Cn, ws.data_ptr(), out.data_ptr(), 0, _stream())
    return out


ACCUM_PARAM_GRADS = os.environ.get("BMC_ACCUM_GRADS", "1") != "0"


def is_sink(p):
    if not (ACCUM_PARAM_GRADS and p is not None and p.is_leaf and p.requires_grad and p.is_contiguous()):
        return False
    if p._backward_hooks:
        return False
    post = p._post_accumulate_grad_hooks
    if post and not set(post.keys()) <= getattr(p, "_bmc_sink_hooks", _NO_HOOKS):
        return False
    return True


_NO_HOOKS = frozenset()


def set_accumulate_param_grads(on: bool):
    global ACCUM_PARAM_GRADS
    ACCUM_PARAM_GRADS = bool(on)


def sink_group(params, full=True):
    if not all(is_sink(p) for p in params):
        return None
    if _SIDE and torch._C._current_graph_task_id() < 0:
        wgrad_join()
    for p in params:
        p._bmc_sink_touched = True
    missing = [p.grad is None for p in params]
    if all(missing) and full:
        for p in params:
            p.grad = torch.empty_like(p, memory_format=torch.contiguous_format)
        acc = 0
    else:
        for p, m in zip(params, missing):
            if m:
                p.grad = torch.zeros_like(p, memory_format=torch.contiguous_format)
            elif not p.grad.is_contiguous():
                p.grad = p.grad.contiguous()
        acc = 1
        if any(missing) and _STREAM_OVERRIDE is not None:
            _SIDE[_cur_dev()].follow_main()
    return [p.grad for p in params], acc


def small_mm(terms, nbatch, bpg, M, N, K, c=None, alpha=1.0, uv=None, vec_out=None, accumulate=False):
    a = lib.SmallMmArgs()
    a.nterms = len(terms)
    for i, (A, B, w) in enumerate(terms):
        t = a.t[i]
        t.a, t.a_sb, t.a_sg, t.a_si, t.a_sk = A[0].data_ptr(), A[1], A[2], A[3], A[4]
        t.b, t.b_sb, t.b_sg, t.b_sk, t.b_sj = B[0].data_ptr(), B[1], B[2], B[3], B[4]
        if w is not None:
            t.w, t.w_sb, t.w_sg, t.w_sk = w[0].data_ptr(), w[1], w[2], w[3]
    a.nbatch, a.batch_per_group, a.M, a.N, a.K, a.alpha = nbatch, bpg, M, N, K, alpha
    if uv is not None:
        (u, usb, usg), (v, vsb, vsg) = uv
        a.u, a.u_sb, a.u_sg, a.v, a.v_sb, a.v_sg = u.data_ptr(), usb, usg, v.data_ptr(), vsb, vsg
    if c is not None:
        a.c, a.c_sb, a.c_sg, a.c_si, a.c_sj = c[0].data_ptr(), c[1], c[2], c[3], c[4]
    if vec_out is not None:
        a.vec_out, a.vo_sb, a.vo_sg = vec_out[0].data_ptr(), vec_out[1], vec_out[2]
    a.accumulate = int(accumulate)
    lib.call(lib._small_mm, "bmc_small_mm", C.byref(a), _stream())


WGRAD_SIDE = os.environ.get("BMC_WGRAD_STREAM", "auto")
WGRAD_SIDE_MIN_PIXELS = int(os.environ.get("BMC_WGRAD_STREAM_MIN_PIXELS", 1 << 14))
if "BMC_WGRAD_STREAM_MAX_PIXELS" in os.environ:
    import warnings
    warnings.warn("BMC_WGRAD_STREAM_MAX_PIXELS is no longer read: the side stream has no upper size limit; "
                  "BMC_WGRAD_KEEP_MAX_PIXELS sets the keep / record_stream threshold of its operands")
WGRAD_KEEP_MAX_PIXELS = int(os.environ.get("BMC_WGRAD_KEEP_MAX_PIXELS", 1 << 17))


class _SideState:
    __slots__ = ("stream", "raw", "event", "keep", "armed", "side", "task", "dev")

    def __init__(self, dev):
        self.dev = dev
        h = C.c_void_p()
        lib.call(lib._stream_low, "bmc_stream_create_low_priority", C.byref(h))
        self.stream = torch.cuda.ExternalStream(h.value, device=dev)
        self.raw = self.stream.cuda_stream
        self.event = torch.cuda.Event()
        self.keep, self.armed, self.side, self.task = [], False, False, -1

    def follow_main(self):
        self.event.record(torch.cuda.current_stream(self.dev))
        self.stream.wait_event(self.event)

    def join(self):
        if self.side:
            torch.cuda.current_stream(self.dev).wait_stream(self.stream)
        self.keep.clear()
        self.armed = False


_SIDE = {}


def wgrad_join():
    cur = torch._C._current_graph_task_id()
    if cur < 0 and _MERGE:
        _MERGE.clear()
    if cur < 0:
        _FLUSH_QUEUED.clear()
    for st in _SIDE.values():
        if st.armed and (cur < 0 or st.task != cur):
            st.join()


def _join_before_step(*_):
    wgrad_join()


from torch.optim.optimizer import register_optimizer_step_pre_hook as _reg_pre_step
_reg_pre_step(_join_before_step)


class _SideCtx:
    __slots__ = ("st",)

    def __init__(self, st):
        self.st = st

    def __enter__(self):
        global _STREAM_OVERRIDE, _STREAM_OVERRIDE_TS
        self.st.follow_main()
        _STREAM_OVERRIDE, _STREAM_OVERRIDE_TS = self.st.raw, self.st.stream
        return self.st

    def __exit__(self, *exc):
        global _STREAM_OVERRIDE, _STREAM_OVERRIDE_TS
        _STREAM_OVERRIDE = _STREAM_OVERRIDE_TS = None
        return False


class _NoCtx:
    def __enter__(self):
        return None

    def __exit__(self, *exc):
        return False


_NOCTX = _NoCtx()



def _side_arm(npx):
    if WGRAD_SIDE == "0" or torch._C._current_graph_task_id() < 0:
        return None
    dev = _cur_dev()
    st = _SIDE.get(dev)
    if st is None:
        st = _SIDE[dev] = _SideState(dev)
    task = torch._C._current_graph_task_id()
    if st.armed and st.task != task:
        st.join()
    if not st.armed:
        st.task = task
        st.side = WGRAD_SIDE == "1" or (MATH == 0 and npx >= WGRAD_SIDE_MIN_PIXELS and not torch.cuda.is_current_stream_capturing())
        _queue_flush(task)
        torch.autograd.Variable._execution_engine.queue_callback(st.join)
        st.armed = True
    return st


def wgrad_side(npx, params, keep=()):
    st = _side_arm(npx)
    if st is None or not st.side:
        return _NOCTX
    ps = [p for p in params if p is not None]
    if not ps or not all(is_sink(p) for p in ps):
        return _NOCTX
    if npx <= WGRAD_KEEP_MAX_PIXELS:
        st.keep.extend(keep)
    else:
        for t in keep:
            t.record_stream(st.stream)
    return _SideCtx(st)


def _flat_params(*ps):
    out = []
    for p in ps:
        if isinstance(p, (tuple, list)):
            out.extend(p)
        elif p is not None:
            out.append(p)
    return out


def reduce_wgrad(slabs, nsplit, G, taps, Cout, spec, dev, bias_slabs, w_param, b_param, w_shape):
    want_b = bias_slabs is not None
    full = spec.covers_all
    if isinstance(w_param, (tuple, list)):
        ps = list(w_param) + (list(b_param) if want_b else [])
        sg = sink_group(ps, full) if 1 < G <= 4 and len(w_param) == G else None
        if sg is not None:
            grads, acc = sg
            PA = C.c_void_p * G
            dwp = PA(*[g.data_ptr() for g in grads[:G]])
            dbp = PA(*[g.data_ptr() for g in grads[G:]]) if want_b else None
            lib.call(lib._red_wg, "bmc_pgemm_reduce_weight_groups", slabs.data_ptr(), nsplit, G, taps, Cout, spec.kpad,
                     spec.kmap(dev).data_ptr(), spec.cin, dwp, acc, bias_slabs.data_ptr() if want_b else None, dbp, _stream())
            return None, None
        w_param = b_param = None
    sg = sink_group([w_param, b_param] if want_b else [w_param], full) if G == 1 and w_param is not None else None
    if sg is not None:
        (gw, *rest), acc = sg
        gb = rest[0] if want_b else None
        lib.call(lib._red_w, "bmc_pgemm_reduce_weight", slabs.data_ptr(), nsplit, 1, taps, Cout, spec.kpad,
                 spec.kmap(dev).data_ptr(), spec.cin, gw.data_ptr(), acc, bias_slabs.data_ptr() if want_b else None,
                 gb.data_ptr() if want_b else None, _stream())
        return None, None
    dw = (torch.empty if full else torch.zeros)(G * Cout * spec.cin * taps, device=dev, dtype=torch.float32)
    db = torch.empty((G, Cout), device=dev, dtype=torch.float32) if want_b else None
    lib.call(lib._red_w, "bmc_pgemm_reduce_weight", slabs.data_ptr(), nsplit, G, taps, Cout, spec.kpad,
             spec.kmap(dev).data_ptr(), spec.cin, dw.data_ptr(), 0, bias_slabs.data_ptr() if want_b else None,
             db.data_ptr() if want_b else None, _stream())
    return dw.view(w_shape), ((db[0] if G == 1 else db) if want_b else None)


class ConvMeta:
    __slots__ = ("spec", "views", "B", "relu", "G", "res", "cache", "taps", "out", "ngp", "rule")

    def __init__(self, spec, views, B, relu, G, res, cache, taps, out=None, ngp=0, rule=None):
        self.spec, self.views, self.B, self.relu, self.G, self.res, self.cache, self.taps, self.out, self.ngp, self.rule = \
            spec, views, B, relu, G, res, cache, taps, out, ngp, rule


class ConvFn(torch.autograd.Function):

    @staticmethod
    def forward(ctx, meta: ConvMeta, weight, bias, res_t, *rest):
        src_ts, gps = (rest[:len(rest) - meta.ngp], rest[len(rest) - meta.ngp:]) if meta.ngp else (rest, ())
        for t in src_ts:
            _need_gpu(t)
        t0 = src_ts[0]
        _, H, W, _ = t0.shape
        G, taps, B = meta.G, meta.taps, meta.B
        w4 = weight.detach().reshape(G, -1, meta.spec.cin, taps)
        Cout = w4.shape[1]
        ck = weight if meta.cache else None
        if meta.out is not None:
            out = meta.out.t[meta.out.b0:meta.out.b0 + B]
            assert out.shape == (B, H, W, Cout) and out.is_contiguous()
        else:
            out = torch.empty((B, H, W, Cout), device=t0.device, dtype=torch.float32)
        srcs = [_src(t.detach(), *v, B) for t, v in zip(src_ts, meta.views)]
        res = None
        if res_t is not None:
            res = _src(res_t.detach(), 0, Cout, meta.res[0], meta.res[1], 0, B)
        conv_launch(srcs, w4.contiguous(), meta.spec, ck, bias.detach() if bias is not None else None, out, B, relu=meta.relu,
                    residual=res, bpg=B // G, rule=meta.rule if meta.rule is not None else bias)
        ctx.meta = meta
        ctx.params = (weight, bias)
        if meta.ngp:
            ctx.params = (tuple(gps[:G]), tuple(gps[G:]) if len(gps) > G else None)
        ctx.w_owner = ck
        ctx.has_bias = bias is not None
        ctx.has_res = res_t is not None
        ctx.window = current_window()
        ctx.save_for_backward(weight, out if meta.relu else None, *src_ts)
        return out

    @staticmethod
    def backward(ctx, dy):
        meta = ctx.meta
        weight, out, *src_ts = ctx.saved_tensors
        G, taps, B, spec = meta.G, meta.taps, meta.B, meta.spec
        dy = dy.contiguous()
        g = relu_bwd(dy, out) if meta.relu else dy
        _, H, W, Cout = g.shape
        dev = g.device
        w4 = weight.detach().reshape(G, Cout, spec.cin, taps).contiguous()
        ck = ctx.w_owner
        need = ctx.needs_input_grad
        ngp = meta.ngp
        nsrc = len(src_ts)
        if ngp:
            need = list(need)
            need[1] = any(need[4 + nsrc:4 + nsrc + G])
            need[2] = any(need[4 + nsrc + G:])
        dw = db = dres = None
        bias_done = False
        a_src = _src(g, 0, Cout, 0, None, 0, B)
        if need[1]:
            wb = ctx.has_bias and need[2]
            wp_, bp_ = ctx.params
            dw, db = wgrad(a_src, [_src(t, *v, B) for t, v in zip(src_ts, meta.views)], spec, B, H, W, taps, Cout, dev, wp_, bp_, G=G,
                           w_shape=weight.shape, keep=(g, *src_ts), window=ctx.window, metas=meta.views, want_bias=wb, merge_pgemm=False)
            if isinstance(dw, list):
                dw = None if all(o is None for o in dw) else torch.stack([
                    o if o is not None else torch.zeros_like(wp_[i]) for i, o in enumerate(dw)])
                db = None if (not wb or all(o is None for o in db)) else torch.stack([
                    o if o is not None else torch.zeros_like(bp_[i]) for i, o in enumerate(db)])
            bias_done = wb
        if ctx.has_bias and need[2] and not bias_done:
            bpg = B // G
            parts = [colsum(g.data_ptr() + 4 * gi * bpg * H * W * Cout, bpg * H * W, Cout, Cout, dev) for gi in range(G)]
            db = parts[0] if G == 1 else torch.stack(parts)
        if ctx.has_res and need[3]:
            shift, mod = meta.res
            dres = g
            if mod is not None and mod < B:
                dres = group_sum(g, B // mod)
            elif shift:
                dres = torch.roll(g, shifts=shift, dims=0)
        shared_dx = {}
        simple = lambda v: v[2] == 0 and v[3] is None
        for i, (t, v) in enumerate(zip(src_ts, meta.views)):
            if need[4 + i] and simple(v):
                shared_dx.setdefault(id(t), []).append(i)
        for key, idxs in list(shared_dx.items()):
            t = src_ts[idxs[0]]
            Bt, _, _, Ct = t.shape
            wins = [(meta.views[i][4], meta.views[i][0], meta.views[i][1]) for i in idxs]
            apart = lambda p, q: p[0] + B <= q[0] or q[0] + B <= p[0] or p[1] + p[2] <= q[1] or q[1] + q[2] <= p[1]
            disjoint = all(apart(wins[j], wins[k]) for j in range(len(wins)) for k in range(j + 1, len(wins)))
            inside = all(w[0] + B <= Bt and w[1] + w[2] <= Ct for w in wins)
            if len(idxs) >= 2 and G == 1 and disjoint and inside and sum(B * w[2] for w in wins) == Bt * Ct:
                shared_dx[key] = (idxs, torch.empty_like(t))
            else:
                del shared_dx[key]
        dsrcs = []
        for i, (t, v) in enumerate(zip(src_ts, meta.views)):
            if not need[4 + i]:
                dsrcs.append(None)
                continue
            grp = shared_dx.get(id(t)) if simple(v) else None
            c0, nch, shift, mod, b0 = v
            Bt, _, _, Ct = t.shape
            if grp is not None:
                dgrad_launch(a_src, w4, spec, i, ck, grp[1], B, out_b0=b0, out_c0=c0)
                dsrcs.append(grp[1] if i == grp[0][0] else None)
                continue
            if G > 1 and ((mod is not None and mod < B) or shift):
                tmp = torch.empty((B, H, W, nch), device=dev, dtype=torch.float32)
                dgrad_launch(a_src, w4, spec, i, ck, tmp, B, bpg=B // G)
                if mod is not None and mod < B:
                    tmp = tmp.view(B // mod, mod, H, W, nch).sum(0)
                    if shift:
                        tmp = torch.roll(tmp, shifts=shift, dims=0)
                elif shift:
                    tmp = torch.roll(tmp, shifts=shift, dims=0)
                nbt = tmp.shape[0]
                if c0 == 0 and nch == Ct and b0 == 0 and nbt == Bt:
                    dx = tmp
                else:
                    dx = torch.zeros_like(t)
                    dx[b0:b0 + nbt, :, :, c0:c0 + nch] = tmp
                dsrcs.append(dx)
                continue
            gs, nb, gshift, gmod = g, B, 0, None
            if mod is not None and mod < B:
                assert shift == 0
                gs, nb = group_sum(g, B // mod), mod
            elif shift:
                assert mod == B
                gshift, gmod = (mod - shift) % mod, mod
            full = (c0 == 0 and nch == Ct and b0 == 0 and nb == Bt)
            dx = torch.empty_like(t) if full else torch.zeros_like(t)
            if Cout % CK:
                raise RuntimeError("bmc_hip: conv output channels must be a multiple of 16 for the data gradient")
            dgrad_launch(_src(gs, 0, Cout, gshift, gmod, 0, nb), w4, spec, i, ck, dx, nb, bpg=nb // G, out_b0=b0, out_c0=c0)
            dsrcs.append(dx)
        if ngp:
            wps, bps = ctx.params
            gw = [None] * G if dw is None else [dw[i].reshape(wps[i].shape) for i in range(G)]
            gb = [] if bps is None else ([None] * G if db is None else [db[i] for i in range(G)])
            return (None, None, None, dres, *dsrcs, *gw, *gb)
        return (None, dw, db, dres, *dsrcs)


def conv(views: Sequence[View], weight, bias, spec: ConvSpec, *, B=None, relu=False, residual=None, G=1,
         cache=True, taps=None, out=None, rule=None):
    B = views[0].t.shape[0] if B is None else B
    if taps is None:
        taps = weight.shape[-1] * weight.shape[-2] if weight.dim() >= 4 else 1
    res_t, res_meta = None, None
    if residual is not None:
        res_t, res_meta = residual.t, (residual.shift, residual.mod)
    meta = ConvMeta(spec, [v.meta() for v in views], B, relu, G, res_meta, cache, taps, out, rule=rule)
    return ConvFn.apply(meta, weight, bias, res_t, *[v.t for v in views])


def conv_groups(views: Sequence[View], weights, biases, spec: ConvSpec, *, B=None, relu=False, residual=None, out=None):
    G = len(weights)
    B = views[0].t.shape[0] if B is None else B
    w0 = weights[0]
    taps = w0.shape[-1] * w0.shape[-2]
    wst = stacked(tuple(weights), lambda: torch.stack([w.detach() for w in weights]), "stack")
    bst = stacked(tuple(biases), lambda: torch.stack([b.detach() for b in biases]), "stack") if biases is not None else None
    res_t, res_meta = None, None
    if residual is not None:
        res_t, res_meta = residual.t, (residual.shift, residual.mod)
    gps = tuple(weights) + (tuple(biases) if biases is not None else ())
    meta = ConvMeta(spec, [v.meta() for v in views], B, relu, G, res_meta, True, taps, out, ngp=len(gps),
                    rule=tuple(biases) if biases is not None else None)
    return ConvFn.apply(meta, wst, bst, res_t, *[v.t for v in views], *gps)


def _wgrad_plain(g, x, spec, w_param, b_param, taps, window=None):
    B, H, W, Cout = g.shape
    return wgrad(_src(g, 0, Cout, 0, None, 0, B), [_src(x, 0, x.shape[3], 0, None, 0, B)], spec, B, H, W, taps, Cout, g.device, w_param,
                 b_param, keep=(g, x), window=window, merge_pgemm=True)


class GradPair:
    __slots__ = ("n", "shape", "buf", "taken")

    def __init__(self, n, shape):
        self.n, self.shape, self.buf, self.taken = n, tuple(shape), None, [False, False]

    def half(self, i, like):
        if self.taken[i]:
            return torch.empty_like(like)
        self.taken[i] = True
        if self.buf is None:
            self.buf = torch.empty(self.shape, device=like.device, dtype=like.dtype)
        return self.buf[i * self.n:(i + 1) * self.n]


def grad_slot(tag, like):
    if tag is None:
        return torch.empty_like(like)
    pair, i = tag
    t = pair.half(i, like)
    return t if t.shape == like.shape else torch.empty_like(like)


class OutSlot:
    __slots__ = ("t", "b0")

    def __init__(self, t, b0):
        self.t, self.b0 = t, b0


class ResBlockFn(torch.autograd.Function):
    @staticmethod
    def forward(ctx, x, w1, b1, w2, b2, spec, out=None):
        _need_gpu(x)
        B, H, W, Cn = x.shape
        taps = w1.shape[-1] * w1.shape[-2]
        xs = _src(x.detach(), 0, Cn, 0, None, 0, B)
        t = torch.empty_like(x)
        conv_launch([xs], w1.detach().reshape(1, Cn, Cn, taps), spec, w1, b1.detach(), t, B, relu=True, rule=b1)
        y = torch.empty_like(x) if out is None else out.t[out.b0:out.b0 + B]
        conv_launch([_src(t, 0, Cn, 0, None, 0, B)], w2.detach().reshape(1, Cn, Cn, taps), spec, w2, b2.detach(), y, B, residual=xs, rule=b2)
        ctx.save_for_backward(x, t, w1, w2)
        ctx.spec, ctx.taps = spec, taps
        ctx.owners = (w1, w2)
        ctx.params = (w1, b1, w2, b2)
        ctx.gslot = getattr(x, "_bmc_gslot", None)
        ctx.window = current_window()
        return y

    @staticmethod
    def backward(ctx, g):
        x, t, w1, w2 = ctx.saved_tensors
        spec, taps = ctx.spec, ctx.taps
        g = g.contiguous()
        B, H, W, Cn = g.shape
        need = ctx.needs_input_grad
        gs, ts = _src(g, 0, Cn, 0, None, 0, B), _src(t, 0, Cn, 0, None, 0, B)
        p_w1, p_b1, p_w2, p_b2 = ctx.params
        dw2, db2 = _wgrad_plain(g, t, spec, p_w2, p_b2, taps, ctx.window) if (need[3] or need[4]) else (None, None)
        dt = torch.empty_like(g)
        dgrad_launch(gs, w2.detach().reshape(1, Cn, Cn, taps), spec, 0, ctx.owners[1], dt, B, mask=ts)
        dts = _src(dt, 0, Cn, 0, None, 0, B)
        dw1, db1 = _wgrad_plain(dt, x, spec, p_w1, p_b1, taps, ctx.window) if (need[1] or need[2]) else (None, None)
        dx = None
        if need[0]:
            dx = grad_slot(ctx.gslot, g)
            dgrad_launch(dts, w1.detach().reshape(1, Cn, Cn, taps), spec, 0, ctx.owners[0], dx, B, residual=gs)
        return dx, dw1, db1, dw2, db2, None, None


def res_block(x, w1, b1, w2, b2, spec, out=None):
    return ResBlockFn.apply(x, w1, b1, w2, b2, spec, out)


class LayerNormFn(torch.autograd.Function):
    @staticmethod
    def forward(ctx, x, gamma, beta, eps):
        _need_gpu(x)
        x = x.contiguous()
        Cn = x.shape[-1]
        npix = x.numel() // Cn
        y = torch.empty_like(x)
        stats = torch.empty(npix * 2, device=x.device, dtype=torch.float32)
        lib.call(lib._ln_fwd, "bmc_layernorm_fwd", x.data_ptr(), gamma.data_ptr(), beta.data_ptr(), npix, Cn, eps,
                 y.data_ptr(), stats.data_ptr(), _stream())
        ctx.save_for_backward(x, stats, gamma)
        ctx.params = (gamma, beta)
        return y

    @staticmethod
    def backward(ctx, dy):
        x, stats, gamma = ctx.saved_tensors
        dy = dy.contiguous()
        Cn = x.shape[-1]
        npix = x.numel() // Cn
        dx = torch.empty_like(x)
        ws = torch.empty(2 * 1024 * Cn, device=x.device, dtype=torch.float32)
        sg = sink_group(list(ctx.params))
        if sg is not None:
            (dg, db), acc = sg
            lib.call(lib._ln_bwd, "bmc_layernorm_bwd", dy.data_ptr(), x.data_ptr(), stats.data_ptr(), gamma.data_ptr(), npix,
                     Cn, dx.data_ptr(), ws.data_ptr(), dg.data_ptr(), db.data_ptr(), acc, _stream())
            return dx, None, None, None
        dg = torch.empty(Cn, device=x.device, dtype=torch.float32)
        db = torch.empty(Cn, device=x.device, dtype=torch.float32)
        lib.call(lib._ln_bwd, "bmc_layernorm_bwd", dy.data_ptr(), x.data_ptr(), stats.data_ptr(), gamma.data_ptr(), npix,
                 Cn, dx.data_ptr(), ws.data_ptr(), dg.data_ptr(), db.data_ptr(), 0, _stream())
        return dx, dg, db, None


def layer_norm(x, gamma, beta, eps=1e-6):
    return LayerNormFn.apply(x, gamma, beta, eps)


_ID_SPECS = {}


def _dense_spec(n):
    s = _ID_SPECS.get(n)
    if s is None:
        s = ConvSpec.dense(n)
        _ID_SPECS[n] = s
    return s


class GramFn(torch.autograd.Function):

    @staticmethod
    def forward(ctx, c, v, scale):
        _need_gpu(c)
        B, H, W, Cn = c.shape
        a_src = _src(c.detach(), 0, Cn, 0, None, 0, B)
        slabs, nsplit, G = pgemm_raw(a_src, [_src(v.detach(), 0, Cn, 0, None, 0, B)], B, H, W, 1, 1, Cn, Cn, c.device,
                                     flops=2.0 * B * H * W * Cn * Cn)
        att = torch.empty((B, Cn, Cn), device=c.device, dtype=torch.float32)
        lib.call(lib._red_p, "bmc_pgemm_reduce_plain", slabs.data_ptr(), nsplit, G, Cn, Cn, scale, att.data_ptr(),
                 _stream())
        ctx.save_for_backward(c, v)
        ctx.scale = scale
        return att

    @staticmethod
    def backward(ctx, datt):
        c, v = ctx.saved_tensors
        B, H, W, Cn = c.shape
        spec = _dense_spec(Cn)
        ds = (datt * ctx.scale).contiguous()
        dc = dv = None
        if ctx.needs_input_grad[0]:
            dc = torch.empty_like(c)
            conv_launch([_src(v, 0, Cn, 0, None, 0, B)], ds.view(B, Cn, Cn, 1), spec, None, None, dc, B, bpg=1)
        if ctx.needs_input_grad[1]:
            dv = torch.empty_like(v)
            conv_launch([_src(c, 0, Cn, 0, None, 0, B)], ds.transpose(1, 2).contiguous().view(B, Cn, Cn, 1), spec, None, None, dv, B, bpg=1)
        return dc, dv, None


def gram(c, v, scale):
    return GramFn.apply(c, v, scale)


class SoftmaxFn(torch.autograd.Function):
    @staticmethod
    def forward(ctx, a):
        _need_gpu(a)
        a = a.contiguous()
        p = torch.empty_like(a)
        Cn = a.shape[-1]
        lib.call(lib._sm_fwd, "bmc_softmax_fwd", a.data_ptr(), a.numel() // Cn, Cn, p.data_ptr(), _stream())
        ctx.save_for_backward(p)
        return p

    @staticmethod
    def backward(ctx, dp):
        (p,) = ctx.saved_tensors
        dp = dp.contiguous()
        Cn = p.shape[-1]
        da = torch.empty_like(p)
        lib.call(lib._sm_bwd, "bmc_softmax_bwd", p.data_ptr(), dp.data_ptr(), p.numel() // Cn, Cn, 1.0, da.data_ptr(),
                 _stream())
        return da


def softmax_rows(a):
    return SoftmaxFn.apply(a)


def attn_apply(p, v, residual: Optional[View] = None):
    B, _, _, Cn = v.shape
    return conv([View(v)], p, None, _dense_spec(Cn), B=B, residual=residual, G=B, cache=False, taps=1)


def pack_inputs(x, repeat=3):
    _need_gpu(x)
    B, _, _, H, W = x.shape
    xin = torch.empty((2 * B, H, W, CK), device=x.device, dtype=torch.float32)
    sb, sc, st, sy, sx = x.stride()
    lib.call(lib._pack_in, "bmc_pack_inputs", x.data_ptr(), sb, sc, st, sy, sx, B, H, W, repeat, xin.data_ptr(),
             xin.data_ptr() + 4 * B * H * W * CK, _stream())
    return xin


def _unshuffle(hr, r, split=1):
    B, Cc, HH, WW = hr.shape
    H, W = HH // r, WW // r
    lr = torch.empty((split * B, H, W, Cc * r * r // split), device=hr.device, dtype=torch.float32)
    lib.call(lib._unshuffle, "bmc_unshuffle_to_nhwc", hr.data_ptr(), B, Cc, H, W, r, lr.data_ptr(), split, _stream())
    return lr


def _shuffle(lr, r, base=None, split=1):
    Bs, H, W, cg = lr.shape
    B, CC = Bs // split, cg * split
    Cc = CC // (r * r)
    hr = torch.empty((B, Cc, H * r, W * r), device=lr.device, dtype=torch.float32)
    if base is None:
        lib.call(lib._shuffle, "bmc_shuffle_to_hr", lr.data_ptr(), B, Cc, H, W, r, None, 0, 0, 0, 0, hr.data_ptr(), split,
                 _stream())
    else:
        sb, sc, sy, sx = base.stride()
        lib.call(lib._shuffle, "bmc_shuffle_to_hr", lr.data_ptr(), B, Cc, H, W, r, base.data_ptr(), sb, sc, sy, sx,
                 hr.data_ptr(), split, _stream())
    return hr


class UnshuffleFn(torch.autograd.Function):

    @staticmethod
    def forward(ctx, hr, r, split):
        _need_gpu(hr)
        ctx.r, ctx.split = r, split
        return _unshuffle(hr.contiguous(), r, split)

    @staticmethod
    def backward(ctx, dlr):
        return _shuffle(dlr.contiguous(), ctx.r, None, ctx.split), None, None


class HeadFn(torch.autograd.Function):

    @staticmethod
    def forward(ctx, xo, base, r):
        _need_gpu(xo)
        ctx.r = r
        return _shuffle(xo.contiguous(), r, base)

    @staticmethod
    def backward(ctx, dpred):
        return _unshuffle(dpred.contiguous(), ctx.r), None, None


class HeadMseFn(torch.autograd.Function):

    @staticmethod
    def forward(ctx, xo, base, gt, r):
        _need_gpu(xo)
        xo = xo.contiguous()
        B, H, W, CC = xo.shape
        Cc = CC // (r * r)
        if tuple(gt.shape) != (B, Cc, H * r, W * r) or not gt.is_cuda or gt.dtype != torch.float32:
            raise RuntimeError("head_mse: ground truth must be a float32 GPU tensor of the prediction's shape")
        if gt.stride()[1:] != (H * r * W * r, W * r, 1):
            gt = gt.contiguous()
        pred = torch.empty((B, Cc, H * r, W * r), device=xo.device, dtype=torch.float32)
        ws = torch.empty(2048, device=xo.device, dtype=torch.float32)
        loss = torch.empty((), device=xo.device, dtype=torch.float32)
        sb, sc, sy, sx = base.stride()
        lib.call(lib._head_mse_fwd, "bmc_head_mse_fwd", xo.data_ptr(), B, Cc, H, W, r, base.data_ptr(), sb, sc, sy, sx,
                 gt.data_ptr(), gt.stride(0), pred.data_ptr(), ws.data_ptr(), loss.data_ptr(), _stream())
        ctx.r = r
        ctx.dims = (B, Cc, H, W)
        ctx.save_for_backward(pred, gt)
        return pred, loss

    @staticmethod
    def backward(ctx, dpred, dloss):
        pred, gt = ctx.saved_tensors
        B, Cc, H, W = ctx.dims
        r = ctx.r
        if dpred is not None:
            dpred = dpred.contiguous()
        if dloss is not None:
            dloss = dloss.contiguous()
        dlr = torch.empty((B, H, W, Cc * r * r), device=pred.device, dtype=torch.float32)
        lib.call(lib._head_mse_bwd, "bmc_head_mse_bwd", dpred.data_ptr() if dpred is not None else None, pred.data_ptr(),
                 gt.data_ptr(), gt.stride(0), dloss.data_ptr() if dloss is not None else None, B, Cc, H, W, r,
                 dlr.data_ptr(), _stream())
        return dlr, None, None, None


def head_mse(xo, base, gt, r):
    return HeadMseFn.apply(xo, base, gt, r)


def pixel_unshuffle_nhwc(hr, r, split=1):
    return UnshuffleFn.apply(hr, r, split)


class StackViewsFn(torch.autograd.Function):

    @staticmethod
    def forward(ctx, *parts):
        p0 = parts[0]
        B, Cc, H, W = p0.shape
        ctx.nb = [p.shape[0] for p in parts]
        out = torch.empty(0, device=p0.device, dtype=p0.dtype)
        out.set_(p0.untyped_storage(), p0.storage_offset(), (sum(ctx.nb), H, W, Cc), (H * W * Cc, W * Cc, Cc, 1))
        return out

    @staticmethod
    def backward(ctx, g):
        outs, b = [], 0
        for n in ctx.nb:
            outs.append(g[b:b + n].permute(0, 3, 1, 2))
            b += n
        return tuple(outs)


def stack_states(parts):
    p0 = parts[0]
    B, Cc, H, W = p0.shape
    want = (H * W * Cc, 1, W * Cc, Cc)
    ok = all(p.is_cuda and p.dtype == torch.float32 and tuple(p.shape[1:]) == (Cc, H, W) and p.stride() == want for p in parts)
    if ok:
        off = p0.storage_offset()
        for p in parts:
            if p.untyped_storage().data_ptr() != p0.untyped_storage().data_ptr() or p.storage_offset() != off:
                ok = False
                break
            off += p.shape[0] * H * W * Cc
    if ok:
        return StackViewsFn.apply(*parts)
    return torch.cat([p.permute(0, 2, 3, 1).contiguous() for p in parts], 0)


def head(xo, base, r):
    return HeadFn.apply(xo, base, r)


class BicubicResizeFn(torch.autograd.Function):

    @staticmethod
    def forward(ctx, x, Ho, Wo):
        _need_gpu(x)
        x = x.contiguous()
        B, Cc, H, W = x.shape
        y = torch.empty((B, Cc, Ho, Wo), device=x.device, dtype=torch.float32)
        lib.call(lib._bicubic_fwd, "bmc_bicubic_resize_fwd", x.data_ptr(), B * Cc, H, W, Ho, Wo, y.data_ptr(), _stream())
        ctx.shape = (B, Cc, H, W)
        return y

    @staticmethod
    def backward(ctx, gy):
        B, Cc, H, W = ctx.shape
        gy = gy.contiguous()
        gx = torch.empty((B, Cc, H, W), device=gy.device, dtype=torch.float32)
        lib.call(lib._bicubic_bwd, "bmc_bicubic_resize_bwd", gy.data_ptr(), B * Cc, H, W, gy.shape[2], gy.shape[3],
                 gx.data_ptr(), _stream())
        return gx, None, None


def bicubic_resize(x, size):
    if tuple(x.shape[-2:]) == (int(size[0]), int(size[1])):
        return x
    return BicubicResizeFn.apply(x, int(size[0]), int(size[1]))


def events_to_channels_batched(xs, ys, ps, offsets, H, W, mutate=True):
    _need_gpu(xs)
    nframes = offsets.numel() - 1
    out = torch.empty((nframes, 2, H, W), device=xs.device, dtype=torch.float32)
    ws = _binned_ws(xs.numel(), nframes, H, W, xs.device)
    if ws is not None:
        lib.call(lib._events_binned, "bmc_events_to_channels_binned", xs.data_ptr(), ys.data_ptr(), ps.data_ptr(),
                 offsets.data_ptr(), xs.numel(), nframes, H, W, out.data_ptr(), int(mutate), ws.data_ptr(), ws.numel() * 8,
                 _stream())
        return out
    lib.call(lib._events, "bmc_events_to_channels", xs.data_ptr(), ys.data_ptr(), ps.data_ptr(), offsets.data_ptr(),
             nframes, H, W, out.data_ptr(), int(mutate), _stream())
    return out


BINNED_MIN_PIXELS = int(os.environ.get("BMC_BINNED_MIN_PIXELS", 1 << 17))


def _binned_ws(nevents, nframes, H, W, device):
    if H * W < BINNED_MIN_PIXELS or nevents == 0 or nframes == 0 or W > 16384:
        return None
    nbytes = lib._events_ws(nevents, nframes, H, W)
    if nbytes < 0:
        return None
    return torch.empty((nbytes + 7) // 8, device=device, dtype=torch.int64)


def encode_raw_events(xs_i16, ys_i16, ps_f64, offsets, flips, H, W):
    for t, dt in ((xs_i16, torch.int16), (ys_i16, torch.int16), (ps_f64, torch.float64), (offsets, torch.int64)):
        if not t.is_cuda or t.dtype != dt or not t.is_contiguous():
            raise RuntimeError("encode_raw_events: expected contiguous %s tensors on the GPU (no CPU fallback)" % dt)
    nframes = offsets.numel() - 1
    out = torch.empty((nframes, 2, H, W), device=xs_i16.device, dtype=torch.float32)
    fp = None
    if flips is not None:
        if flips.dtype != torch.uint8 or not flips.is_cuda or flips.numel() != nframes:
            raise RuntimeError("encode_raw_events: flips must be a uint8 GPU vector with one entry per frame")
        fp = flips.data_ptr()
    ws = _binned_ws(xs_i16.numel(), nframes, H, W, xs_i16.device)
    if ws is not None:
        lib.call(lib._enc_raw_binned, "bmc_encode_raw_events_binned", xs_i16.data_ptr(), ys_i16.data_ptr(), ps_f64.data_ptr(),
                 offsets.data_ptr(), fp, xs_i16.numel(), nframes, H, W, out.data_ptr(), ws.data_ptr(), ws.numel() * 8, _stream())
        return out
    lib.call(lib._enc_raw, "bmc_encode_raw_events", xs_i16.data_ptr(), ys_i16.data_ptr(), ps_f64.data_ptr(),
             offsets.data_ptr(), fp, nframes, H, W, out.data_ptr(), _stream())
    return out


def events_to_voxel_batched(xs, ys, ts, ps, offsets, bins, H, W, mutate=True):
    _need_gpu(xs)
    nframes = offsets.numel() - 1
    n = xs.numel()
    out = torch.empty((nframes, bins, H, W), device=xs.device, dtype=torch.float32)
    ws = torch.empty(2 * nframes * (H * W + 1) + n, device=xs.device, dtype=torch.int32)
    lib.call(lib._voxel, "bmc_events_to_voxel", xs.data_ptr(), ys.data_ptr(), ts.data_ptr(), ps.data_ptr(),
             offsets.data_ptr(), n, nframes, bins, H, W, out.data_ptr(), int(mutate), ws.data_ptr(), _stream())
    return out


def _bin_bounds(ts, bins):
    dt = ts[-1] - ts[0] + 1e-6
    delta_t = dt / bins
    bi = torch.arange(bins, device=ts.device, dtype=torch.float32)
    tstart = ts[0] + delta_t * bi
    return tstart, tstart + delta_t


def events_to_stack_polarity(xs, ys, ts, ps, bins, H, W, mutate=True):
    _need_gpu(xs)
    tstart, tend = _bin_bounds(ts, bins)
    out = torch.empty((2, bins, H, W), device=xs.device, dtype=torch.float32)
    ranges = torch.empty(2 * bins, device=xs.device, dtype=torch.int32)
    lib.call(lib._stack_pol, "bmc_events_to_stack_polarity", xs.data_ptr(), ys.data_ptr(), ts.data_ptr(), ps.data_ptr(),
             ts.numel(), tstart.data_ptr(), tend.data_ptr(), bins, H, W, out.data_ptr(), ranges.data_ptr(), int(mutate),
             _stream())
    return out


def events_to_mask(xs, ys, ps, H, W, mutate=True):
    _need_gpu(xs)
    out = torch.empty((H, W), device=xs.device, dtype=torch.float32)
    ws = torch.empty(H * W, device=xs.device, dtype=torch.int32)
    lib.call(lib._mask, "bmc_events_to_mask", xs.data_ptr(), ys.data_ptr(), ps.data_ptr(), xs.numel(), H, W, out.data_ptr(),
             ws.data_ptr(), int(mutate), _stream())
    return out


def events_to_stack(xs, ys, ts, ps, bins, H, W, mutate=True):
    _need_gpu(xs)
    n = ts.numel()
    dt = ts[-1] - ts[0] + 1e-6
    delta_t = dt / bins
    bi = torch.arange(bins, device=ts.device, dtype=torch.float32)
    tstart = ts[0] + delta_t * bi
    tend = tstart + delta_t
    out = torch.empty((bins, H, W), device=xs.device, dtype=torch.float32)
    ranges = torch.empty(2 * bins, device=xs.device, dtype=torch.int32)
    lib.call(lib._stack, "bmc_events_to_stack", xs.data_ptr(), ys.data_ptr(), ts.data_ptr(), ps.data_ptr(), n,
             tstart.data_ptr(), tend.data_ptr(), bins, H, W, out.data_ptr(), ranges.data_ptr(), int(mutate), _stream())
    return out
```

### include/bmc_hip.h

```cpp
#ifndef BMC_HIP_H
#define BMC_HIP_H

#ifdef __cplusplus
extern "C" {
#endif

typedef void* bmc_stream_t;

#define BMC_MAX_SRC 6
#define BMC_CK 16

typedef struct bmc_src {
    const float* ptr;
    long long batch_stride;
    int pix_stride;
    int nch;
    int batch_shift;
    int batch_mod;
} bmc_src_t;
#define BMC_SRC_TABLE (-1)


int bmc_version(void);
const char* bmc_last_error(void);
int bmc_stream_create_low_priority(bmc_stream_t* out);

int bmc_events_to_channels(float* xs, float* ys, const float* ps, const long long* offsets,
                           int nframes, int H, int W, float* out, int mutate, bmc_stream_t s);

long long bmc_events_binned_ws_bytes(long long nevents, int nframes, int H, int W);
int bmc_events_to_channels_binned(float* xs, float* ys, const float* ps, const long long* offsets, long long nevents,
                                  int nframes, int H, int W, float* out, int mutate, void* ws, long long ws_bytes,
                                  bmc_stream_t s);
int bmc_encode_raw_events_binned(const short* xs, const short* ys, const double* ps, const long long* offsets,
                                 const unsigned char* flips, long long nevents, int nframes, int H, int W, float* out,
                                 void* ws, long long ws_bytes, bmc_stream_t s);

long long bmc_events_torch_ws_ints(long long n, int H, int W);
int bmc_events_to_image_torch(float* xs, float* ys, float* ps, long long n, int H, int W, int clip_out_of_range, int bilinear,
                              int padding, float* out, int* ws, bmc_stream_t s);
int bmc_events_to_voxel_torch(float* xs, float* ys, const float* ts, const float* ps, long long n, int bins, int H, int W,
                              float* out, int* ws, bmc_stream_t s);

int bmc_events_to_voxel(float* xs, float* ys, const float* ts, const float* ps, const long long* offsets,
                        long long nevents, int nframes, int bins, int H, int W, float* out, int mutate, int* ws,
                        bmc_stream_t s);

int bmc_events_to_stack(float* xs, float* ys, const float* ts, float* ps, long long n, const float* tstart,
                        const float* tend, int bins, int H, int W, float* out, int* ranges, int mutate, bmc_stream_t s);

int bmc_events_to_stack_polarity(float* xs, float* ys, const float* ts, const float* ps, long long n, const float* tstart,
                                 const float* tend, int bins, int H, int W, float* out, int* ranges, int mutate,
                                 bmc_stream_t s);

int bmc_events_to_mask(float* xs, float* ys, float* ps, long long n, int H, int W, float* out, int* ws, int mutate,
                       bmc_stream_t s);

int bmc_encode_raw_events(const short* xs, const short* ys, const double* ps, const long long* offsets,
                          const unsigned char* flips, int nframes, int H, int W, float* out, bmc_stream_t s);

int bmc_pack_weight(const float* w, const int* kmap, int G, int Cout, int Cin, int taps,
                    int Kpad, int Coutpad, float* out, bmc_stream_t s);
int bmc_pack_weight_t(const float* w, const int* kmap, int G, int Cout, int Cin, int taps,
                      int k0, int nk, int nkpad, int Coutpad16, float* out, bmc_stream_t s);
#define BMC_MATH_FP32 0
#define BMC_MATH_BF16 1
#define BMC_MATH_BF16X6 3
#define BMC_MATH_FP32_WINO 4
#define BMC_MATH_FP32_WINO4 5
int bmc_split_weight(const float* packed, void* out, long long nsteps, int Coutpad, int planes, bmc_stream_t s);

int bmc_pack_weight_wino(const float* w, const int* kmap, int G, int Cout, int Cin, int Kpad, int Coutpad, int transposed,
                         int k0, int nk, float* out, bmc_stream_t s);

int bmc_conv_wino_rows(int B, int H, int W, int Coutpad, int cus);

int bmc_pack_weight_wino4(const float* w, const int* kmap, int G, int Cout, int Cin, int Kpad, int Coutpad, int transposed,
                          int k0, int nk, float* out, bmc_stream_t s);

typedef struct bmc_conv_args {
    int nsrc;
    bmc_src_t src[BMC_MAX_SRC];
    const void* wpacked;
    const float* bias;
    long long w_group_stride;
    int bias_group_stride;
    int batch_per_group;
    float* out;
    long long out_batch_stride;
    int out_pix_stride;
    int B, H, W;
    int Cout, Coutpad;
    int taps;
    int relu;
    bmc_src_t residual;
    bmc_src_t mask;
    int accumulate;
    int math;
} bmc_conv_args_t;
int bmc_conv(const bmc_conv_args_t* host_args, bmc_stream_t s);

typedef struct bmc_pgemm_args {
    bmc_src_t a;
    int nsrc;
    bmc_src_t src[BMC_MAX_SRC];
    int B, H, W, taps;
    int batch_per_group;
    float* slabs;
    int nsplit;
    const float* zeros;
    float* bias_slabs;
    int math;
    int tap_groups;
} bmc_pgemm_args_t;
int bmc_pgemm(const bmc_pgemm_args_t* host_args, bmc_stream_t s);
int bmc_pgemm_wave_map(int taps, int M, int N);
int bmc_pgemm_reduce_weight(const float* slabs, int nsplit, int G, int taps, int M, int N, const int* kmap,
                            int Cin, float* dw, int accumulate, const float* bias_slabs ,
                            float* db , bmc_stream_t s);
int bmc_pgemm_reduce_weight_groups(const float* slabs, int nsplit, int G, int taps, int M, int N, const int* kmap,
                                   int Cin, float* const* dw, int accumulate, const float* bias_slabs, float* const* db,
                                   bmc_stream_t s);
int bmc_pgemm_reduce_plain(const float* slabs, int nsplit, int G, int M, int N, float scale,
                           float* out, bmc_stream_t s);

int bmc_wgrad_wino_nsplit(int B, int H, int W);
int bmc_wgrad_wino(const bmc_src_t* dy, const bmc_src_t* x, int B, int H, int W, int nsplit, float* part, float* bias_part,
                   bmc_stream_t s);
int bmc_wgrad_wino_reduce(const float* part, int nsplit, float* dw, int ldw, int k0, int accumulate, const float* bias_part,
                          float* db, bmc_stream_t s);
int bmc_wgrad_wino_multi(const bmc_src_t* dy, const bmc_src_t* x, const int* batches, int nseg, int H, int W, int nsplit,
                         float* part, float* bias_part, bmc_stream_t s);

int bmc_wgrad_wino4_nsplit(int B, int H, int W);
int bmc_wgrad_wino4(const bmc_src_t* dy, const bmc_src_t* x, int B, int H, int W, int nsplit, float* part, float* bias_part,
                    bmc_stream_t s);
int bmc_wgrad_wino4_reduce(const float* part, int nsplit, float* dw, int ldw, int k0, int accumulate, const float* bias_part,
                           float* db, bmc_stream_t s);

int bmc_ptr_table(const unsigned long long* ptrs, int n, unsigned long long* table, bmc_stream_t s);

int bmc_group_sum(const float* in, int groups, long long n, float* out, bmc_stream_t s);
int bmc_colsum(const float* x, long long npix, int pix_stride, int C, float* ws, float* out,
               int accumulate, bmc_stream_t s);
int bmc_relu_bwd(const float* dy, const float* y, float* g, long long n, bmc_stream_t s);
int bmc_layernorm_fwd(const float* x, const float* gamma, const float* beta, long long npix, int C,
                      float eps, float* y, float* stats, bmc_stream_t s);
int bmc_layernorm_bwd(const float* dy, const float* x, const float* stats, const float* gamma,
                      long long npix, int C, float* dx, float* ws, float* dgamma, float* dbeta,
                      int accumulate, bmc_stream_t s);
int bmc_softmax_fwd(const float* a, long long rows, int C, float* p, bmc_stream_t s);
int bmc_softmax_bwd(const float* p, const float* dp, long long rows, int C, float scale_out,
                    float* da, bmc_stream_t s);

int bmc_pack_inputs(const float* x, long long sb, long long sc, long long st, long long sy, long long sx,
                    int B, int H, int W, int repeat, float* xin_p, float* xin_n, bmc_stream_t s);
int bmc_unshuffle_to_nhwc(const float* hr, int B, int C, int H, int W, int r, float* lr, int split, bmc_stream_t s);
int bmc_shuffle_to_hr(const float* lr, int B, int C, int H, int W, int r, const float* base,
                      long long sb, long long sc, long long sy, long long sx, float* hr, int split ,
                      bmc_stream_t s);

int bmc_head_mse_fwd(const float* lr, int B, int C, int H, int W, int r, const float* base, long long sb, long long sc,
                     long long sy, long long sx, const float* gt, long long gt_batch_stride, float* hr, float* partials,
                     float* loss, bmc_stream_t s);
int bmc_head_mse_bwd(const float* dpred, const float* pred, const float* gt, long long gt_batch_stride, const float* gloss,
                     int B, int C, int H, int W, int r, float* dlr, bmc_stream_t s);

typedef struct bmc_chain_fwd_args {
    bmc_src_t s0, s1;
    const float* wstream;
    const float* bias_f;
    const float* bias_c;
    const float* gamma;
    const float* beta;
    float eps;
    float* yhat;
    float* rstd;
    float* centre;
    int B, C, H, W;
} bmc_chain_fwd_args_t;
int bmc_chain_fwd(const bmc_chain_fwd_args_t* host_args, bmc_stream_t s);

typedef struct bmc_chain_bwd_args {
    bmc_src_t dcentre;
    const float* wstream;
    const float* gamma;
    const float* yhat;
    const float* rstd;
    float* dz;
    float* ds1;
    float* ds0;
    bmc_src_t ds0_add;
    int n, C, H, W;
} bmc_chain_bwd_args_t;
int bmc_chain_bwd(const bmc_chain_bwd_args_t* host_args, bmc_stream_t s);
int bmc_chain_affine_grads(const float* G, const float* dbc, const float* Wc, const float* gamma, const float* beta, int C,
                           float* dwc, float* dbc_out, float* dgamma, float* dbeta, int accumulate, bmc_stream_t s);

typedef struct {
    const float* a; long long a_sb, a_sg; int a_si, a_sk;
    const float* b; long long b_sb, b_sg; int b_sk, b_sj;
    const float* w; long long w_sb, w_sg; int w_sk;
} bmc_mm_term_t;
typedef struct {
    int nterms;
    bmc_mm_term_t t[2];
    int nbatch, batch_per_group;
    int M, N, K;
    float alpha;
    const float* u; long long u_sb, u_sg;
    const float* v; long long v_sb, v_sg;
    float* c; long long c_sb, c_sg; int c_si, c_sj;
    float* vec_out; long long vo_sb, vo_sg;
    int accumulate;
} bmc_small_mm_args_t;
int bmc_small_mm(const bmc_small_mm_args_t* host_args, bmc_stream_t s);

int bmc_bicubic_resize_fwd(const float* x, long long planes, int H, int W, int Ho, int Wo, float* y, bmc_stream_t s);
int bmc_bicubic_resize_bwd(const float* gy, long long planes, int H, int W, int Ho, int Wo, float* gx, bmc_stream_t s);

#define BMC_MAX_SLOTS 256
#define BMC_SLOT_ACTIVE 1
#define BMC_SLOT_RESET 2
typedef struct bmc_slot {
    const float* frames;
    const float* gt;
    float* keep;
    double* result;
    int flags;
    int pad_;
} bmc_slot_t;

int bmc_slot_stage(const bmc_slot_t* table, int S, int seqn, int H, int W, float* x, const void* feat_pool, int pool_bf16,
                   float* feat, int nfeat, long long feat_n, float* pred, long long pred_n, bmc_stream_t s);
int bmc_slot_commit(const bmc_slot_t* table, int S, const float* const* feat_src, int nfeat, long long feat_n, void* feat_pool,
                    int pool_bf16, const float* pred_src, float* pred_pool, long long pred_n, bmc_stream_t s);
#define BMC_SLOT_MAX_PARTS 64
int bmc_slot_metrics(const bmc_slot_t* table, int S, const float* pred, int sH, int sW, int H, int W, int gh, int gw,
                     int nparts, bmc_stream_t s);

#define BMC_SLOT_MAX_SEQN 8
typedef struct bmc_slot_events {
    const short* lr_xs;
    const short* lr_ys;
    const double* lr_ps;
    const short* gt_xs;
    const short* gt_ys;
    const double* gt_ps;
    long long gt_range[2];
    long long lr_range[BMC_SLOT_MAX_SEQN][2];
} bmc_slot_events_t;
int bmc_slot_encode(const bmc_slot_events_t* table, int S, int seqn, int H, int W, int gh, int gw, float* lr_scratch,
                    float* gt_scratch, bmc_stream_t s);

typedef struct bmc_slot_emit {
    short* xs;
    short* ys;
    signed char* ps;
    const long long* index_in;
    long long* index_out;
    long long capacity;
} bmc_slot_emit_t;
#define BMC_SLOT_EMIT_MAX_PARTS 1024
int bmc_slot_emit(const bmc_slot_t* table, const bmc_slot_emit_t* emit, int S, const float* pred, int sH, int sW, int max_count,
                  int nparts, unsigned* parts, bmc_stream_t s);

#define BMC_EVENT_T0 0.01
#define BMC_EVENT_T1 1.0
#define BMC_SLOT_EMIT_TIMED_MAX_COUNT 255
#define BMC_SLOT_EMIT_TIMED_BLOCK 4096
#define BMC_SLOT_EMIT_TIMED_MAX_WINDOW (1ll << 28)
typedef struct bmc_slot_emit_timed {
    short* xs;
    short* ys;
    signed char* ps;
    const long long* index_in;
    long long* index_out;
    long long capacity;
    float* ts;
} bmc_slot_emit_timed_t;
long long bmc_slot_emit_timed_scratch_bytes(int S, int nparts, long long window_capacity);
int bmc_slot_emit_timed(const bmc_slot_t* table, const bmc_slot_emit_timed_t* emit, int S, const float* pred, int sH, int sW,
                        int max_count, int nparts, unsigned* parts, const unsigned short* rank_table, void* scratch,
                        long long window_capacity, bmc_stream_t s);

typedef struct bmc_slot_clock {
    double t_first;
    double t_last;
    double* ts;
} bmc_slot_clock_t;
int bmc_slot_emit_clocked(const bmc_slot_t* table, const bmc_slot_emit_timed_t* emit, const bmc_slot_clock_t* clock, int S,
                          const float* pred, int sH, int sW, int max_count, int nparts, unsigned* parts,
                          const unsigned short* rank_table, void* scratch, long long window_capacity, bmc_stream_t s);

typedef struct bmc_slot_hot {
    int* hot_pixels;
    unsigned char* hot_mask;
    int first_item;
    int new_from;
    int active;
    int pad_;
    int cmin[BMC_SLOT_MAX_SEQN];
} bmc_slot_hot_t;
int bmc_slot_hot_update(const bmc_slot_hot_t* hot, const bmc_slot_events_t* events, int S, int seqn, int H, int W, int max_px,
                        int negative_rate, int* counts, unsigned char* ring, int* ws, bmc_stream_t s);
int bmc_slot_encode_filtered(const bmc_slot_events_t* table, const bmc_slot_hot_t* hot, const unsigned char* ring, int S, int seqn,
                             int H, int W, int gh, int gw, float* lr_scratch, float* gt_scratch, bmc_stream_t s);
int bmc_hot_pixel_mask(float* event_rate, int H, int W, int active, int max_px, float max_rate, float* mask, unsigned* ws,
                       bmc_stream_t s);

#define BMC_SLOT_RENDER_MAX_PIXELS (1 << 24)
#define BMC_SLOT_RENDER_MAX_PARTS 1024
typedef struct bmc_slot_render {
    const float* src;
    unsigned char* dst;
} bmc_slot_render_t;
int bmc_slot_render(const bmc_slot_t* table, const bmc_slot_render_t* render, int S, int h, int w, int round, int nparts,
                    float* scratch, bmc_stream_t s);

#ifdef __cplusplus
}
#endif
#endif
```

Baseline: 47.70 LR-voxel-frames/s.

## Fuse BIE channel-attention reduce, softmax and value-weight products into single kernels

Adds fused HIP kernels for the value-free channel attention in the BIE blocks. The forward kernel reduces the Gram slabs, applies the value weights and bias, runs the softmax and writes the attention-times-weight matrix straight into the packed 1x1 conv weight layout. The backward kernel does the same for the gradient path, including softmax backward and building the packed dc/dx weights. This replaces a chain of small_mm, reduce, softmax and packing launches plus intermediate tensors with one launch per direction, aimed at launch overhead and memory traffic on small matrices. It adds a new packed-weight bypass in conv_launch and only applies when MATH==0 and C is at most 128.

```diff
diff --git a/bmcnet-esr_amd/bmc_hip/bie.py b/bmcnet-esr_amd/bmc_hip/bie.py
--- a/bmcnet-esr_amd/bmc_hip/bie.py
+++ b/bmcnet-esr_amd/bmc_hip/bie.py
@@ -22,6 +22,46 @@
 
 def vfree_supported(npx):
     return VFREE and ops.MATH in (0, 3) and npx >= VFREE_MIN_PIXELS
+
+
+FUSE_ATTN = os.environ.get("BMC_FUSE_ATTN", "1") != "0"
+
+
+def attn_fused(Cn):
+    return FUSE_ATTN and ops.MATH == 0 and Cn % 16 == 0 and Cn <= 128
+
+
+def attn_fwd(c_src, x_src, nb, H, W, Cn, wg, bg, bpg, scale, dev):
+    slabs, nsplit, G, bsl = pgemm_raw(c_src, [x_src], nb, H, W, 1, 1, Cn, Cn, dev, flops=2.0 * nb * H * W * Cn * Cn, want_bias=True)
+    new = lambda *shape: torch.empty(shape, device=dev, dtype=torch.float32)
+    G0, sc, p, pb, pwp = new(nb, Cn, Cn), new(nb, Cn), new(nb, Cn, Cn), new(nb, Cn), new(nb * Cn * ops.coutpad(Cn))
+    a = lib.BieAttnFwdArgs()
+    a.slabs, a.bias_slabs, a.nsplit = slabs.data_ptr(), bsl.data_ptr(), nsplit
+    a.wv, a.bv, a.batch_per_group, a.scale = wg.data_ptr(), bg.data_ptr(), bpg, scale
+    a.nb, a.C = nb, Cn
+    a.g0, a.s, a.p, a.pb, a.pw_packed = G0.data_ptr(), sc.data_ptr(), p.data_ptr(), pb.data_ptr(), pwp.data_ptr()
+    lib.call(lib._bie_attn_fwd, "bmc_bie_attn_fwd", C.byref(a), _stream())
+    return G0, sc, p, pb, pwp
+
+
+def attn_bwd(g_src, x_src, n_att, nb, H, W, Cn, p, pwp, wg, bg, bpg, w_ut, scale, dev):
+    slabs, nsplit, G, bsl = pgemm_raw(g_src, [x_src], n_att, H, W, 1, 1, Cn, Cn, dev, flops=2.0 * n_att * H * W * Cn * Cn, want_bias=True)
+    new = lambda *shape: torch.empty(shape, device=dev, dtype=torch.float32)
+    cp = ops.coutpad(Cn)
+    dM, tg, da, ds = new(n_att, Cn, Cn), new(n_att, Cn), new(n_att, Cn, Cn), new(nb, Cn)
+    w_dc, w_dx = new(nb * 2 * Cn * cp), new(n_att * 2 * Cn * cp)
+    a = lib.BieAttnBwdArgs()
+    a.slabs, a.bias_slabs, a.nsplit = slabs.data_ptr(), bsl.data_ptr(), nsplit
+    a.p, a.pw_packed = p.data_ptr(), pwp.data_ptr()
+    a.wv, a.bv, a.batch_per_group, a.w_ut, a.batch_per_half, a.scale = wg.data_ptr(), bg.data_ptr(), bpg, w_ut.data_ptr(), nb // 2, scale
+    a.nb, a.n_att, a.C = nb, n_att, Cn
+    a.dm, a.t, a.da, a.ds, a.w_dc, a.w_dx = dM.data_ptr(), tg.data_ptr(), da.data_ptr(), ds.data_ptr(), w_dc.data_ptr(), w_dx.data_ptr()
+    lib.call(lib._bie_attn_bwd, "bmc_bie_attn_bwd", C.byref(a), _stream())
+    return dM, tg, da, ds, w_dc, w_dx
+
+
+def _w_ut2(p_wu, wu, Cn):
+    return ops.stacked((p_wu,), lambda: wu.detach().view(Cn, 2, Cn).permute(1, 2, 0).contiguous(), "wut")
 
 
 def _gram_on_x(c_src, x_src, B, H, W, Cn, dev):
@@ -177,7 +217,13 @@
         bv = ops.stacked((bv1, bv2), lambda: torch.stack([d(bv1), d(bv2)]), "stack")
         vfree = vfree_supported(B2 * H * W)
         o12 = new(B2)
-        if vfree:
+        fattn = vfree and attn_fused(Cn)
+        pwp = None
+        if fattn:
+            v12 = None
+            G0, sc, p, pb, pwp = attn_fwd(X(c12), X(x12), B2, H, W, Cn, wv.view(2, Cn, Cn), bv, n, scale, dev)
+            conv_launch([X(x12)], (B2, Cn, Cn, 1), s1, None, pb, o12, B2, residual=X(r12, shift=n, mod=B2), bpg=1, packed=pwp)
+        elif vfree:
             G0, sc = _gram_on_x(X(c12), X(x12), B2, H, W, Cn, dev)
             wg, v12 = wv.view(2, Cn, Cn), None
             att = _times_wt(G0, sc, wg, bv, n, scale, torch.empty_like(G0))
@@ -199,8 +245,9 @@
         xs_new = new(n)
         conv_launch([X(c12, b0=0, B=n), X(c12, b0=n, B=n)], d(wu).reshape(1, Cn, 2 * Cn, 1), s2, wu, d(bu), xs_new, n, residual=X(xs))
         ctx.save_for_backward(x12, xs, t12, z12, stats, y12, c12, v12 if not vfree else G0, p, rw1, rw2, wf, gamma, wc, wu, wv1, wv2, beta,
-                              *((sc, bv1, bv2) if vfree else ()))
+                              *((sc, bv1, bv2) if vfree else ()), *((pwp,) if fattn else ()))
         ctx.vfree = vfree
+        ctx.fattn = fattn
         ctx.owners = (rw1, rw2, wf, wc, wu)
         ctx.window = ops.current_window()
         ctx.params = (rw1, rb1, rw2, rb2, wf, bf, gamma, beta, wc, bc, wu, bu)
@@ -215,8 +262,9 @@
         saved = ctx.saved_tensors
         x12, xs, t12, z12, stats, y12, c12, v12, p, rw1, rw2, wf, gamma, wc, wu, wv1, wv2, beta = saved[:18]
         vfree = ctx.vfree
-        if vfree:
-            G0, (sc, bv1, bv2) = v12, saved[18:]
+        fattn = ctx.fattn
+        if vfree:
+            G0, (sc, bv1, bv2) = v12, saved[18:21]
         o_rw1, o_rw2, o_wf, o_wc, o_wu = ctx.owners
         p_rw1, p_rb1, p_rw2, p_rb2, p_wf, p_bf, p_gamma, p_beta, p_wc, p_bc, p_wu, p_bu = ctx.params
         B2, H, W, Cn = x12.shape
@@ -234,19 +282,27 @@
         if vfree:
             wg = w_v.view(2, Cn, Cn)
             bg = ops.stacked(ctx.vparams[2:], lambda: torch.stack([bv1.detach(), bv2.detach()]), "stack")
-            dM, tg = _gram_on_x(X(g_o), X(x12), B2, H, W, Cn, dev)
-            dp = _times_wt(dM, tg, wg, bg, n, 1.0, torch.empty_like(dM))
+            if fattn:
+                dM, tg, da, ds, w_dc, w_dx = attn_bwd(X(g_o), X(x12), B2, B2, H, W, Cn, p, saved[21], wg, bg, n,
+                                                      _w_ut2(p_wu, wu, Cn), ctx.scale, dev)
+            else:
+                dM, tg = _gram_on_x(X(g_o), X(x12), B2, H, W, Cn, dev)
+                dp = _times_wt(dM, tg, wg, bg, n, 1.0, torch.empty_like(dM))
         else:
             slabs, nsplit, G = pgemm_raw(X(g_o), [X(v12)], B2, H, W, 1, 1, Cn, Cn, dev, flops=2.0 * B2 * H * W * Cn * Cn)
             dp = torch.empty_like(p)
             lib.call(lib._red_p, "bmc_pgemm_reduce_plain", slabs.data_ptr(), nsplit, G, Cn, Cn, 1.0, dp.data_ptr(), _stream())
-        da = torch.empty_like(p)
-        lib.call(lib._sm_bwd, "bmc_softmax_bwd", p.data_ptr(), dp.data_ptr(), B2 * Cn, Cn, ctx.scale, da.data_ptr(), _stream())
+        if not fattn:
+            da = torch.empty_like(p)
+            lib.call(lib._sm_bwd, "bmc_softmax_bwd", p.data_ptr(), dp.data_ptr(), B2 * Cn, Cn, ctx.scale, da.data_ptr(), _stream())
         if vfree:
             dwv, dbv = _value_param_grads(p, dM, tg, da, G0, sc, ctx.vparams[:2], ctx.vparams[2:], B2 * H * W)
         dc12 = new(B2)
-        w_ut = ops.stacked((p_wu,), lambda: wu.detach().view(Cn, 2, Cn).permute(1, 2, 0).repeat_interleave(n, 0).contiguous(), "wut%d" % n)
-        if vfree:
+        w_ut = None if fattn else ops.stacked((p_wu,), lambda: wu.detach().view(Cn, 2, Cn).permute(1, 2, 0).repeat_interleave(n, 0).contiguous(), "wut%d" % n)
+        w2 = (B2, Cn, 2 * Cn, 1)
+        if fattn:
+            conv_launch([X(x12), X(g_x, mod=n, B=B2)], w2, s2, None, ds, dc12, B2, bpg=1, packed=w_dc)
+        elif vfree:
             w_dx = torch.empty((B2, Cn, 2 * Cn, 1), device=dev, dtype=torch.float32)
             w_dc = torch.empty((B2, Cn, 2 * Cn, 1), device=dev, dtype=torch.float32)
             w_dc.view(B2, Cn, 2 * Cn)[:, :, Cn:] = w_ut
@@ -285,13 +341,14 @@
             dwf, dbf = ops.wgrad(X(dz12), [X(xs, mod=n, B=B2), X(x12, shift=n, mod=B2)], s2, B2, H, W, 1, Cn, dev, p_wf, p_bf,
                               keep=(dz12, xs, x12), window=ctx.window, merge_pgemm=True)
             if vfree:
-                conv_launch([X(g_o), X(c12)], w_dx, s2, None, None, dx12, B2, bpg=1, accumulate=True)
+                conv_launch([X(g_o), X(c12)], w2 if fattn else w_dx, s2, None, None, dx12, B2, bpg=1, accumulate=True,
+                            packed=w_dx if fattn else None)
             else:
                 dgrad_launch(X(dv12), w_v, s1, 0, w_v, dx12, B2, bpg=n, accumulate=True)
         else:
             dx12 = ops.grad_slot(ctx.gslot, x12)
             if vfree:
-                conv_launch([X(g_o), X(c12)], w_dx, s2, None, None, dx12, B2, bpg=1)
+                conv_launch([X(g_o), X(c12)], w2 if fattn else w_dx, s2, None, None, dx12, B2, bpg=1, packed=w_dx if fattn else None)
             else:
                 dgrad_launch(X(dv12), w_v, s1, 0, w_v, dx12, B2, bpg=n)
             dwc, dbc = ops.wgrad(X(dc12), [X(y12)], s1, B2, H, W, 1, Cn, dev, p_wc, p_bc, keep=(dc12, y12), window=ctx.window, merge_pgemm=True)
@@ -347,7 +404,14 @@
                                     B2, H, W, Cn, dev)
         vfree = vfree_supported(B2 * H * W)
         o1 = new(n)
-        if vfree:
+        fattn = vfree and attn_fused(Cn)
+        pwp = None
+        if fattn:
+            v1 = None
+            G0, sc, p, pb, pwp = attn_fwd(X(c12, b0=0, B=n), X(x12, b0=0, B=n), n, H, W, Cn, d(wv1).reshape(1, Cn, Cn).contiguous(),
+                                          d(bv1).reshape(1, Cn).contiguous(), n, scale, dev)
+            conv_launch([X(x12, b0=0, B=n)], (n, Cn, Cn, 1), s1, None, pb, o1, n, residual=X(r2), bpg=1, packed=pwp)
+        elif vfree:
             G0, sc = _gram_on_x(X(c12, b0=0, B=n), X(x12, b0=0, B=n), n, H, W, Cn, dev)
             wg, bg, v1 = d(wv1).reshape(1, Cn, Cn), d(bv1).reshape(1, Cn), None
             att = _times_wt(G0, sc, wg, bg, n, scale, torch.empty_like(G0))
@@ -369,8 +433,9 @@
         xs_new = new(n)
         conv_launch([X(c12, b0=0, B=n), X(c12, b0=n, B=n)], d(wu).reshape(1, Cn, 2 * Cn, 1), s2, wu, d(bu), xs_new, n, residual=X(xs))
         ctx.save_for_backward(x12, xs, t2, yhat, rstd, c12, v1 if not vfree else G0, p, rw1, rw2, wf, gamma, wc, wu, wv1, beta,
-                              *((sc, bv1) if vfree else ()))
+                              *((sc, bv1) if vfree else ()), *((pwp,) if fattn else ()))
         ctx.vfree = vfree
+        ctx.fattn = fattn
         ctx.owners = (rw1, rw2, wf, wc, wu, wv1)
         ctx.window = ops.current_window()
         ctx.params = (rw1, rb1, rw2, rb2, wf, bf, gamma, beta, wc, bc, wu, bu, wv1, bv1)
@@ -382,8 +447,9 @@
         saved = ctx.saved_tensors
         x12, xs, t2, yhat, rstd, c12, v1, p, rw1, rw2, wf, gamma, wc, wu, wv1, beta = saved[:16]
         vfree = ctx.vfree
-        if vfree:
-            G0, (sc, bv1) = v1, saved[16:]
+        fattn = ctx.fattn
+        if vfree:
+            G0, (sc, bv1) = v1, saved[16:18]
         o_rw1, o_rw2, o_wf, o_wc, o_wu, o_wv1 = ctx.owners
         p_rw1, p_rb1, p_rw2, p_rb2, p_wf, p_bf, p_gamma, p_beta, p_wc, p_bc, p_wu, p_bu, p_wv1, p_bv1 = ctx.params
         B2, H, W, Cn = x12.shape
@@ -398,21 +464,28 @@
         w_v1 = wv1.detach().reshape(1, Cn, Cn, 1)
         if vfree:
             wg, bg = wv1.detach().reshape(1, Cn, Cn), bv1.detach().reshape(1, Cn)
-            dM, tg = _gram_on_x(X(g_o), X(x12, b0=0, B=n), n, H, W, Cn, dev)
-            dp = _times_wt(dM, tg, wg, bg, n, 1.0, torch.empty_like(dM))
+            if fattn:
+                dM, tg, da, ds, w_dc, w_dx = attn_bwd(X(g_o), X(x12, b0=0, B=n), n, B2, H, W, Cn, p, saved[18], wg.contiguous(),
+                                                      bg.contiguous(), n, _w_ut2(p_wu, wu, Cn), ctx.scale, dev)
+            else:
+                dM, tg = _gram_on_x(X(g_o), X(x12, b0=0, B=n), n, H, W, Cn, dev)
+                dp = _times_wt(dM, tg, wg, bg, n, 1.0, torch.empty_like(dM))
         else:
             slabs, nsplit, G = pgemm_raw(X(g_o), [X(v1)], n, H, W, 1, 1, Cn, Cn, dev, flops=2.0 * n * H * W * Cn * Cn)
             dp = torch.empty_like(p)
             lib.call(lib._red_p, "bmc_pgemm_reduce_plain", slabs.data_ptr(), nsplit, G, Cn, Cn, 1.0, dp.data_ptr(), _stream())
-        da = torch.empty_like(p)
-        lib.call(lib._sm_bwd, "bmc_softmax_bwd", p.data_ptr(), dp.data_ptr(), n * Cn, Cn, ctx.scale, da.data_ptr(), _stream())
+        if not fattn:
+            da = torch.empty_like(p)
+            lib.call(lib._sm_bwd, "bmc_softmax_bwd", p.data_ptr(), dp.data_ptr(), n * Cn, Cn, ctx.scale, da.data_ptr(), _stream())
         if vfree:
             dwv1, dbv1 = _value_param_grads(p, dM, tg, da, G0, sc, (p_wv1,), (p_bv1,), n * H * W)
             if dwv1 is not None:
                 dwv1, dbv1 = dwv1.view(wv1.shape), dbv1.view(Cn)
         dc12 = new(B2)
-        w_ut = ops.stacked((p_wu,), lambda: wu.detach().view(Cn, 2, Cn).permute(1, 2, 0).repeat_interleave(n, 0).contiguous(), "wut%d" % n)
-        if vfree:
+        w_ut = None if fattn else ops.stacked((p_wu,), lambda: wu.detach().view(Cn, 2, Cn).permute(1, 2, 0).repeat_interleave(n, 0).contiguous(), "wut%d" % n)
+        if fattn:
+            conv_launch([X(x12), X(g_x, mod=n, B=B2)], (B2, Cn, 2 * Cn, 1), s2, None, ds, dc12, B2, bpg=1, packed=w_dc)
+        elif vfree:
             w_dx = torch.empty((n, Cn, 2 * Cn, 1), device=dev, dtype=torch.float32)
             w_dc = torch.zeros((B2, Cn, 2 * Cn, 1), device=dev, dtype=torch.float32)
             w_dc.view(B2, Cn, 2 * Cn)[:, :, Cn:] = w_ut
@@ -448,7 +521,8 @@
         dwf, dbf = ops.wgrad(X(dz12), [X(xs, mod=n, B=B2), X(x12, shift=n, mod=B2)], s2, B2, H, W, 1, Cn, dev, p_wf, p_bf,
                           keep=(dz12, xs, x12), window=ctx.window, merge_pgemm=True)
         if vfree:
-            conv_launch([X(g_o), X(c12, b0=0, B=n)], w_dx, s2, None, None, dx12, n, bpg=1, accumulate=True)
+            conv_launch([X(g_o), X(c12, b0=0, B=n)], (n, Cn, 2 * Cn, 1) if fattn else w_dx, s2, None, None, dx12, n, bpg=1, accumulate=True,
+                        packed=w_dx if fattn else None)
         else:
             dgrad_launch(X(dv1), w_v1, s1, 0, o_wv1, dx12, n, accumulate=True)
         dw2, db2 = ops.wgrad(X(g_o), [X(t2)], s1, n, H, W, 9, Cn, dev, p_rw2, p_rb2, keep=(g_o, t2), window=ctx.window, merge_pgemm=True)
diff --git a/bmcnet-esr_amd/bmc_hip/lib.py b/bmcnet-esr_amd/bmc_hip/lib.py
--- a/bmcnet-esr_amd/bmc_hip/lib.py
+++ b/bmcnet-esr_amd/bmc_hip/lib.py
@@ -67,6 +67,22 @@
                 ("vec_out", C.c_void_p), ("vo_sb", C.c_longlong), ("vo_sg", C.c_longlong), ("accumulate", C.c_int)]
 
 
+class BieAttnFwdArgs(C.Structure):
+    _fields_ = [("slabs", C.c_void_p), ("bias_slabs", C.c_void_p), ("nsplit", C.c_int),
+                ("wv", C.c_void_p), ("bv", C.c_void_p), ("batch_per_group", C.c_int), ("scale", C.c_float),
+                ("nb", C.c_int), ("C", C.c_int),
+                ("g0", C.c_void_p), ("s", C.c_void_p), ("p", C.c_void_p), ("pb", C.c_void_p), ("pw_packed", C.c_void_p)]
+
+
+class BieAttnBwdArgs(C.Structure):
+    _fields_ = [("slabs", C.c_void_p), ("bias_slabs", C.c_void_p), ("nsplit", C.c_int),
+                ("p", C.c_void_p), ("pw_packed", C.c_void_p),
+                ("wv", C.c_void_p), ("bv", C.c_void_p), ("batch_per_group", C.c_int), ("w_ut", C.c_void_p), ("batch_per_half", C.c_int), ("scale", C.c_float),
+                ("nb", C.c_int), ("n_att", C.c_int), ("C", C.c_int),
+                ("dm", C.c_void_p), ("t", C.c_void_p), ("da", C.c_void_p), ("ds", C.c_void_p), ("w_dc", C.c_void_p),
+                ("w_dx", C.c_void_p)]
+
+
 def _sig(name, argtypes, restype=C.c_int):
     fn = getattr(_lib, name)
     fn.argtypes = argtypes
@@ -97,6 +113,8 @@
 _ww_nsplit = _sig("bmc_wgrad_wino_nsplit", [_i, _i, _i])
 _stream_low = _sig("bmc_stream_create_low_priority", [C.POINTER(C.c_void_p)])
 _small_mm = _sig("bmc_small_mm", [C.POINTER(SmallMmArgs), _p])
+_bie_attn_fwd = _sig("bmc_bie_attn_fwd", [C.POINTER(BieAttnFwdArgs), _p])
+_bie_attn_bwd = _sig("bmc_bie_attn_bwd", [C.POINTER(BieAttnBwdArgs), _p])
 _ww = _sig("bmc_wgrad_wino", [C.POINTER(Src), C.POINTER(Src), _i, _i, _i, _i, _p, _p, _p])
 _ww_red = _sig("bmc_wgrad_wino_reduce", [_p, _i, _p, _i, _i, _i, _p, _p, _p])
 _ww_multi = _sig("bmc_wgrad_wino_multi", [C.POINTER(Src), C.POINTER(Src), C.POINTER(C.c_int), _i, _i, _i, _i, _p, _p, _p])
@@ -155,7 +173,7 @@
            "bmc_wgrad_wino4_nsplit", "bmc_wgrad_wino4", "bmc_wgrad_wino4_reduce", "bmc_wgrad_wino_multi", "bmc_ptr_table",
            "bmc_conv_wino_rows", "bmc_slot_stage", "bmc_slot_commit", "bmc_slot_metrics", "bmc_slot_encode", "bmc_slot_emit",
            "bmc_slot_emit_timed", "bmc_slot_emit_timed_scratch_bytes", "bmc_slot_emit_clocked", "bmc_slot_hot_update",
-           "bmc_slot_encode_filtered", "bmc_hot_pixel_mask", "bmc_slot_render"]
+           "bmc_slot_encode_filtered", "bmc_hot_pixel_mask", "bmc_slot_render", "bmc_bie_attn_fwd", "bmc_bie_attn_bwd"]
 
 
 def check(rc, what):
diff --git a/bmcnet-esr_amd/bmc_hip/ops.py b/bmcnet-esr_amd/bmc_hip/ops.py
--- a/bmcnet-esr_amd/bmc_hip/ops.py
+++ b/bmcnet-esr_amd/bmc_hip/ops.py
@@ -761,11 +761,15 @@
 
 
 def conv_launch(srcs, w4, spec, owner, bias, out, B, relu=False, residual=None, mask=None, bpg=None, accumulate=False,
-                out_b0=0, rule=None):
-    G, Cout, Cin, taps = w4.shape
+                out_b0=0, rule=None, packed=None):
+    G, Cout, Cin, taps = w4 if packed is not None else w4.shape
     _, H, W, Co = out.shape
     wn = wino_ok(B, H, W, Cout, taps, fwd=not accumulate and mask is None, stride=_launch_stride(srcs, Co, residual, mask), rule=rule)
-    wp = _packed_weight(w4, spec, owner, wino=wn)
+    if packed is not None:
+        assert MATH == 0 and taps == 1 and packed.numel() == G * spec.kpad * coutpad(Cout)
+        wp = packed
+    else:
+        wp = _packed_weight(w4, spec, owner, wino=wn)
     conv_raw(srcs, wp, spec.kpad * taps * coutpad(Cout), bias, Cout if bias is not None else 0,
              out.data_ptr() + 4 * out_b0 * H * W * Co, H * W * Co, Co, B, H, W, Cout, taps, relu=relu, residual=residual,
              bpg=bpg, accumulate=accumulate, mask=mask, flops=2.0 * B * H * W * Cout * taps * spec.kreal, wino=wn)
diff --git a/bmcnet-esr_amd/csrc/bie_attn.hip b/bmcnet-esr_amd/csrc/bie_attn.hip
--- /dev/null
+++ b/bmcnet-esr_amd/csrc/bie_attn.hip
@@ -0,0 +1,278 @@
+#include "bmc_common.h"
+
+namespace {
+
+constexpr int R = 16;
+constexpr int CMAX = 128;
+constexpr int NT = 256;
+constexpr int PITCH_MAX = CMAX + 4;
+
+struct FwdK { bmc_bie_attn_fwd_args_t a; };
+struct BwdK { bmc_bie_attn_bwd_args_t a; };
+
+struct Lds {
+    float w[CMAX * PITCH_MAX];
+    float x[R * PITCH_MAX];
+    float p[R * PITCH_MAX];
+    float d[R * PITCH_MAX];
+    float bv[CMAX];
+    float v[R];
+    float red[NT];
+};
+
+__device__ __forceinline__ int coutpad_of(int C) { return C <= 32 ? 32 : 128; }
+
+__device__ __forceinline__ void load_w(Lds& l, const float* W, const float* bvec, int C, int pitch, int tid) {
+    const int c4s = C / 4, nq = C * c4s;
+    for (int q0 = 0; q0 < nq; q0 += 4 * NT) {
+        f32x4 v[4];
+#pragma unroll
+        for (int u = 0; u < 4; ++u) {
+            const int q = q0 + u * NT + tid;
+            if (q < nq) v[u] = ldg16(W + (long long)(q / c4s) * C + (q % c4s) * 4);
+        }
+#pragma unroll
+        for (int u = 0; u < 4; ++u) {
+            const int q = q0 + u * NT + tid;
+            if (q < nq) *reinterpret_cast<f32x4*>(&l.w[(q / c4s) * pitch + (q % c4s) * 4]) = v[u];
+        }
+    }
+    if (tid < C) l.bv[tid] = ldg4(bvec + tid);
+}
+
+__device__ __forceinline__ void reduce_rows(Lds& l, const float* slabs, const float* bias_slabs, int nsplit, int G, int b, int i0,
+                                            int C, int pitch, float* out, float* vec, int tid) {
+    const int pad = (C + 31) / 32 * 32, c4s = C / 4, nq = R * c4s;
+    const long long slab = (long long)G * pad * pad;
+    for (int q = tid; q < nq; q += NT) {
+        const int row = q / c4s, c = (q % c4s) * 4;
+        const float* p = slabs + ((long long)b * pad + i0 + row) * pad + c;
+        f32x4 acc = {0.f, 0.f, 0.f, 0.f};
+        int s = 0;
+        for (; s + 8 <= nsplit; s += 8) {
+            f32x4 v[8];
+#pragma unroll
+            for (int u = 0; u < 8; ++u) v[u] = ldg16(p + (long long)(s + u) * slab);
+#pragma unroll
+            for (int u = 0; u < 8; ++u) acc += v[u];
+        }
+        for (; s < nsplit; ++s) acc += ldg16(p + (long long)s * slab);
+        *reinterpret_cast<f32x4*>(&l.x[row * pitch + c]) = acc;
+        stg16(out + ((long long)b * C + i0 + row) * C + c, acc);
+    }
+    {
+        const int row = tid & (R - 1), part = tid >> 4, n4 = nsplit * 4;
+        auto at = [&](int i) { return ldg4(bias_slabs + (((long long)(i >> 2) * G + b) * 4 + (i & 3)) * pad + i0 + row); };
+        float s = 0.f;
+        int i = part;
+        for (; i + 7 * 16 < n4; i += 8 * 16) {
+            float v[8];
+#pragma unroll
+            for (int u = 0; u < 8; ++u) v[u] = at(i + u * 16);
+#pragma unroll
+            for (int u = 0; u < 8; ++u) s += v[u];
+        }
+        for (; i < n4; i += 16) s += at(i);
+        l.red[tid] = s;
+    }
+    __syncthreads();
+    if (tid < R) {
+        float t = 0.f;
+#pragma unroll
+        for (int k = 0; k < NT / R; ++k) t += l.red[k * R + tid];
+        l.v[tid] = t;
+        stg4(vec + (long long)b * C + i0 + tid, t);
+    }
+}
+
+__device__ __forceinline__ void product_nt(const float* A, const float* Ws, int C, int pitch, int j, int h, float (&acc)[8]) {
+#pragma unroll
+    for (int r = 0; r < 8; ++r) acc[r] = 0.f;
+    for (int k = 0; k < C; k += 4) {
+        const f32x4 w = *reinterpret_cast<const f32x4*>(&Ws[j * pitch + k]);
+#pragma unroll
+        for (int r = 0; r < 8; ++r) {
+            const f32x4 a = *reinterpret_cast<const f32x4*>(&A[(8 * h + r) * pitch + k]);
+#pragma unroll
+            for (int q = 0; q < 4; ++q) acc[r] = fmaf(a[q], w[q], acc[r]);
+        }
+    }
+}
+
+__device__ __forceinline__ void product_nn(const float* A, const float* Ws, int C, int pitch, int k, int h, float (&acc)[8]) {
+#pragma unroll
+    for (int r = 0; r < 8; ++r) acc[r] = 0.f;
+    for (int j = 0; j < C; j += 4) {
+        float w[4];
+#pragma unroll
+        for (int q = 0; q < 4; ++q) w[q] = Ws[(j + q) * pitch + k];
+#pragma unroll
+        for (int r = 0; r < 8; ++r) {
+            const f32x4 a = *reinterpret_cast<const f32x4*>(&A[(8 * h + r) * pitch + j]);
+#pragma unroll
+            for (int q = 0; q < 4; ++q) acc[r] = fmaf(a[q], w[q], acc[r]);
+        }
+    }
+}
+
+__device__ __forceinline__ float wave_sum(float s) {
+#pragma unroll
+    for (int m = 1; m < 64; m <<= 1) s += __shfl_xor(s, m);
+    return s;
+}
+
+__device__ __forceinline__ void zero_pad_rows(float* packed, int nchunks, int C, int cp, int tid) {
+    const int per = (cp - C) * 16;
+    for (int e = tid; e < nchunks * per; e += NT) stg4(packed + ((long long)(e / per) * cp + C) * 16 + e % per, 0.f);
+}
+
+__global__ __launch_bounds__(NT) void bie_attn_fwd_kernel(const FwdK k) {
+    const bmc_bie_attn_fwd_args_t& a = k.a;
+    __shared__ __attribute__((aligned(16))) Lds l;
+    const int tid = threadIdx.x, lane = tid & 63, wave = tid >> 6;
+    const int C = a.C, pitch = C + 4, cp = coutpad_of(C);
+    const int b = blockIdx.y, i0 = blockIdx.x * R, g = b / a.batch_per_group;
+    load_w(l, a.wv + (long long)g * C * C, a.bv + (long long)g * C, C, pitch, tid);
+    reduce_rows(l, a.slabs, a.bias_slabs, a.nsplit, a.nb, b, i0, C, pitch, a.g0, a.s, tid);
+    __syncthreads();
+    const int j = tid & (CMAX - 1), h = tid >> 7;
+    float acc[8];
+    if (j < C) {
+        product_nt(l.x, l.w, C, pitch, j, h, acc);
+#pragma unroll
+        for (int r = 0; r < 8; ++r) l.p[(8 * h + r) * pitch + j] = a.scale * (acc[r] + l.v[8 * h + r] * l.bv[j]);
+    }
+    __syncthreads();
+    for (int row = wave; row < R; row += NT / 64) {
+        float* ar = &l.p[row * pitch];
+        float mx = -INFINITY;
+        for (int c = lane; c < C; c += 64) mx = fmaxf(mx, ar[c]);
+#pragma unroll
+        for (int m = 1; m < 64; m <<= 1) mx = fmaxf(mx, __shfl_xor(mx, m));
+        float s = 0.f;
+        for (int c = lane; c < C; c += 64) s += expf(ar[c] - mx);
+        s = wave_sum(s);
+        const float inv = 1.f / s;
+        float pb = 0.f;
+        for (int c = lane; c < C; c += 64) {
+            const float pv = expf(ar[c] - mx) * inv;
+            ar[c] = pv;
+            stg4(a.p + ((long long)b * C + i0 + row) * C + c, pv);
+            pb = fmaf(pv, l.bv[c], pb);
+        }
+        pb = wave_sum(pb);
+        if (lane == 0) stg4(a.pb + (long long)b * C + i0 + row, pb);
+    }
+    __syncthreads();
+    float* pw = a.pw_packed + (long long)b * C * cp;
+    if (j < C) {
+        product_nn(l.p, l.w, C, pitch, j, h, acc);
+#pragma unroll
+        for (int r = 0; r < 8; ++r) stg4(pw + ((long long)(j >> 4) * cp + i0 + 8 * h + r) * 16 + (j & 15), acc[r]);
+    }
+    if (cp > C && blockIdx.x == 0) zero_pad_rows(pw, C / 16, C, cp, tid);
+}
+
+__global__ __launch_bounds__(NT) void bie_attn_bwd_kernel(const BwdK k) {
+    const bmc_bie_attn_bwd_args_t& a = k.a;
+    __shared__ __attribute__((aligned(16))) Lds l;
+    const int tid = threadIdx.x, lane = tid & 63, wave = tid >> 6;
+    const int C = a.C, pitch = C + 4, cp = coutpad_of(C);
+    const int b = blockIdx.y, i0 = blockIdx.x * R, g = b / a.batch_per_group;
+    float* wdc = a.w_dc + (long long)b * 2 * C * cp;
+    {
+        const float* wut = a.w_ut + ((long long)(b / a.batch_per_half) * C + i0) * C;
+        for (int e = tid; e < R * C; e += NT) {
+            const int c = e % C, row = e / C;
+            stg4(wdc + ((long long)((C + c) >> 4) * cp + i0 + row) * 16 + (c & 15), ldg4(wut + (long long)row * C + c));
+        }
+    }
+    if (cp > C && blockIdx.x == 0) zero_pad_rows(wdc, 2 * C / 16, C, cp, tid);
+    if (b >= a.n_att) {
+        for (int e = tid; e < (C / 16) * R * 16; e += NT)
+            stg4(wdc + ((long long)(e / (R * 16)) * cp + i0) * 16 + e % (R * 16), 0.f);
+        if (tid < R) stg4(a.ds + (long long)b * C + i0 + tid, 0.f);
+        return;
+    }
+    load_w(l, a.wv + (long long)g * C * C, a.bv + (long long)g * C, C, pitch, tid);
+    for (int q = tid; q < R * (C / 4); q += NT) {
+        const int row = q / (C / 4), c = (q % (C / 4)) * 4;
+        *reinterpret_cast<f32x4*>(&l.p[row * pitch + c]) = ldg16(a.p + ((long long)b * C + i0 + row) * C + c);
+    }
+    reduce_rows(l, a.slabs, a.bias_slabs, a.nsplit, a.n_att, b, i0, C, pitch, a.dm, a.t, tid);
+    __syncthreads();
+    const int j = tid & (CMAX - 1), h = tid >> 7;
+    float acc[8];
+    if (j < C) {
+        product_nt(l.x, l.w, C, pitch, j, h, acc);
+#pragma unroll
+        for (int r = 0; r < 8; ++r) l.d[(8 * h + r) * pitch + j] = acc[r] + l.v[8 * h + r] * l.bv[j];
+    }
+    __syncthreads();
+    for (int row = wave; row < R; row += NT / 64) {
+        const float* pr = &l.p[row * pitch];
+        float* dr = &l.d[row * pitch];
+        float s = 0.f;
+        for (int c = lane; c < C; c += 64) s += pr[c] * dr[c];
+        s = wave_sum(s);
+        float sb = 0.f;
+        for (int c = lane; c < C; c += 64) {
+            const float dv = pr[c] * (dr[c] - s) * a.scale;
+            dr[c] = dv;
+            stg4(a.da + ((long long)b * C + i0 + row) * C + c, dv);
+            sb = fmaf(dv, l.bv[c], sb);
+        }
+        sb = wave_sum(sb);
+        if (lane == 0) stg4(a.ds + (long long)b * C + i0 + row, sb);
+    }
+    __syncthreads();
+    float* wdx = a.w_dx + (long long)b * 2 * C * cp;
+    if (j < C) {
+        product_nn(l.d, l.w, C, pitch, j, h, acc);
+#pragma unroll
+        for (int r = 0; r < 8; ++r) stg4(wdc + ((long long)(j >> 4) * cp + i0 + 8 * h + r) * 16 + (j & 15), acc[r]);
+        float* o = wdx + ((long long)((C + i0) >> 4) * cp + j) * 16 + 8 * h;
+        stg16(o, f32x4{acc[0], acc[1], acc[2], acc[3]});
+        stg16(o + 4, f32x4{acc[4], acc[5], acc[6], acc[7]});
+        const float* pw = a.pw_packed + (long long)b * C * cp + ((long long)(j >> 4) * cp + i0 + 8 * h) * 16 + (j & 15);
+#pragma unroll
+        for (int r = 0; r < 8; ++r) acc[r] = ldg4(pw + r * 16);
+        o = wdx + ((long long)(i0 >> 4) * cp + j) * 16 + 8 * h;
+        stg16(o, f32x4{acc[0], acc[1], acc[2], acc[3]});
+        stg16(o + 4, f32x4{acc[4], acc[5], acc[6], acc[7]});
+    }
+    if (cp > C && blockIdx.x == 0) zero_pad_rows(wdx, 2 * C / 16, C, cp, tid);
+}
+
+}
+
+extern "C" int bmc_bie_attn_fwd(const bmc_bie_attn_fwd_args_t* host_args, bmc_stream_t stream) {
+    BMC_CHECK_ARG(host_args, "bmc_bie_attn_fwd: null arguments");
+    const bmc_bie_attn_fwd_args_t& a = *host_args;
+    BMC_CHECK_ARG(a.C >= 16 && a.C <= CMAX && a.C % 16 == 0, "bmc_bie_attn_fwd: C = %d (a multiple of 16, at most %d)", a.C, CMAX);
+    BMC_CHECK_ARG(a.nb >= 1 && a.nb <= 65535 && a.nsplit >= 1 && a.batch_per_group >= 1,
+                  "bmc_bie_attn_fwd: bad sizes (samples %d, per group %d, splits %d)", a.nb, a.batch_per_group, a.nsplit);
+    BMC_CHECK_ARG(a.slabs && a.bias_slabs && a.wv && a.bv && a.g0 && a.s && a.p && a.pb && a.pw_packed, "bmc_bie_attn_fwd: null operand");
+    FwdK k;
+    k.a = a;
+    hipLaunchKernelGGL(bie_attn_fwd_kernel, dim3((unsigned)(a.C / R), (unsigned)a.nb), dim3(NT), 0, (hipStream_t)stream, k);
+    BMC_CHECK_LAUNCH("bmc_bie_attn_fwd");
+    return 0;
+}
+
+extern "C" int bmc_bie_attn_bwd(const bmc_bie_attn_bwd_args_t* host_args, bmc_stream_t stream) {
+    BMC_CHECK_ARG(host_args, "bmc_bie_attn_bwd: null arguments");
+    const bmc_bie_attn_bwd_args_t& a = *host_args;
+    BMC_CHECK_ARG(a.C >= 16 && a.C <= CMAX && a.C % 16 == 0, "bmc_bie_attn_bwd: C = %d (a multiple of 16, at most %d)", a.C, CMAX);
+    BMC_CHECK_ARG(a.nb >= 1 && a.nb <= 65535 && a.n_att >= 1 && a.n_att <= a.nb && a.nsplit >= 1 && a.batch_per_group >= 1 &&
+                      a.batch_per_half >= 1 && (a.nb - 1) / a.batch_per_half <= 1,
+                  "bmc_bie_attn_bwd: bad sizes (samples %d, with attention %d, per group %d, per half %d, splits %d)", a.nb, a.n_att,
+                  a.batch_per_group, a.batch_per_half, a.nsplit);
+    BMC_CHECK_ARG(a.slabs && a.bias_slabs && a.p && a.pw_packed && a.wv && a.bv && a.w_ut && a.dm && a.t && a.da && a.ds && a.w_dc && a.w_dx,
+                  "bmc_bie_attn_bwd: null operand");
+    BwdK k;
+    k.a = a;
+    hipLaunchKernelGGL(bie_attn_bwd_kernel, dim3((unsigned)(a.C / R), (unsigned)a.nb), dim3(NT), 0, (hipStream_t)stream, k);
+    BMC_CHECK_LAUNCH("bmc_bie_attn_bwd");
+    return 0;
+}
diff --git a/include/bmc_hip.h b/include/bmc_hip.h
--- a/include/bmc_hip.h
+++ b/include/bmc_hip.h
@@ -216,6 +216,25 @@
 } bmc_small_mm_args_t;
 int bmc_small_mm(const bmc_small_mm_args_t* host_args, bmc_stream_t s);
 
+typedef struct {
+    const float* slabs; const float* bias_slabs; int nsplit;
+    const float* wv; const float* bv; int batch_per_group;
+    float scale;
+    int nb, C;
+    float* g0; float* s; float* p; float* pb; float* pw_packed;
+} bmc_bie_attn_fwd_args_t;
+int bmc_bie_attn_fwd(const bmc_bie_attn_fwd_args_t* host_args, bmc_stream_t s);
+typedef struct {
+    const float* slabs; const float* bias_slabs; int nsplit;
+    const float* p; const float* pw_packed;
+    const float* wv; const float* bv; int batch_per_group;
+    const float* w_ut; int batch_per_half;
+    float scale;
+    int nb, n_att, C;
+    float* dm; float* t; float* da; float* ds; float* w_dc; float* w_dx;
+} bmc_bie_attn_bwd_args_t;
+int bmc_bie_attn_bwd(const bmc_bie_attn_bwd_args_t* host_args, bmc_stream_t s);
+
 int bmc_bicubic_resize_fwd(const float* x, long long planes, int H, int W, int Ho, int Wo, float* y, bmc_stream_t s);
 int bmc_bicubic_resize_bwd(const float* gy, long long planes, int H, int W, int Ho, int Wo, float* gx, bmc_stream_t s);
 
```

New measurement: 47.42 LR-voxel-frames/s. About the same (-0.6%).
